# YuliangXiu/ICON

Hardware: NVIDIA H100
Metric: M query-points/sec at 256^3 grid (higher is better)
Workload: dtype f32

## Files before the change

icon_b200/_C.py:

```python
import ctypes
import os

_HERE = os.path.dirname(os.path.abspath(__file__))
LIB_PATH = os.environ.get("ICON_B200_LIB") or os.path.join(_HERE, "libicon_b200.so")

if not os.path.exists(LIB_PATH):
    raise ImportError(
        f"{LIB_PATH} is missing: the CUDA extension must be built (python -m icon_b200.build); "
        "icon_b200 has no CPU or PyTorch fallback.")

lib = ctypes.CDLL(LIB_PATH)

_vp, _i, _i64, _f, _sz = ctypes.c_void_p, ctypes.c_int, ctypes.c_int64, ctypes.c_float, ctypes.c_size_t

_SIGS = {
    "icon_version": (_i, []),
    "icon_last_error": (ctypes.c_char_p, []),
    "icon_launch_count": (_i64, []),
    "icon_profile_enable": (_i, [_i]),
    "icon_profile_last_query": (_i, [_vp]),
    "icon_smpl_workspace_bytes": (_sz, [_i, _i]),
    "icon_smpl_prepare": (_i, [_vp, _vp, _vp, _vp, _i, _i, _vp, _sz, _vp]),
    "icon_query_workspace_bytes": (_sz, [_i64, _i, _i]),
    "icon_set_mlp_impl": (_i, [_i]),
    "icon_get_mlp_impl": (_i, []),
    "icon_query": (_i, [_i, _vp, _i64, _i64, _i64, _vp, _vp, _i, _i, _i, _vp, _i, _vp, _i, _i, _vp, _vp, _i, _f,
                        _vp, _vp, _sz, _vp]),
    "icon_query_feats": (_i, [_i, _vp, _i64, _i64, _i64, _vp, _vp, _i, _i, _i, _vp, _i, _vp, _i, _i, _vp, _vp, _i, _f,
                              _i, _vp, _vp, _sz, _vp]),
    "icon_set_sdf_policy": (_i, [_i, _i64, _i64]),
    "icon_set_sdf_bricks": (_i, [_i, _i64]),
    "icon_sdf_brick_info": (_i, [_vp, _i, _i, _vp]),
    "icon_sdf_brick_lists": (_i, [_vp, _i, _i, _vp, _vp, _vp, _vp, _vp, _vp, _vp]),
    "icon_sdf_only": (_i, [_vp, _i64, _i64, _i64, _vp, _vp, _i, _i, _vp, _vp, _vp, _sz, _vp]),
    "icon_sdf_bruteforce": (_i, [_vp, _i64, _i64, _i64, _vp, _vp, _i, _i, _vp, _vp, _vp]),
    "icon_face_tree_read": (_i, [_vp, _i, _i, _vp, _vp, _vp, _vp]),
    "icon_mesh_workspace_bytes": (_sz, [_i, _i]),
    "icon_mesh_prepare": (_i, [_vp, _vp, _i, _i, _vp, _sz, _vp]),
    "icon_mesh_distance": (_i, [_vp, _i64, _vp, _i, _i, _vp, _vp, _vp]),
    "icon_mesh_sample_workspace_bytes": (_sz, [_i]),
    "icon_mesh_sample": (_i, [_vp, _vp, _i, _i, _vp, _i, ctypes.c_uint64, _vp, _vp, _vp, _vp, _sz, _vp]),
    "icon_prt_workspace_bytes": (_sz, [_i, _i, _i]),
    "icon_prt": (_i, [_vp, _i, _i, _vp, _vp, _i, ctypes.c_double, _vp, _vp, _i, _i, ctypes.c_double, _vp, _vp, _vp, _sz,
                      _vp]),
    "icon_mlp_only": (_i, [_vp, _i, _i64, _vp, _vp, _vp, _vp]),
    "icon_display": (_i, [_vp, _i, _vp, _vp]),
    "icon_grid_upsample": (_i, [_vp, _vp, _i, _f, _vp, _vp, _vp, _vp]),
    "icon_grid_dilate": (_i, [_vp, _i, _i, _vp, _vp, _vp]),
    "icon_compact_workspace_bytes": (_sz, [_i]),
    "icon_grid_compact": (_i, [_vp, _vp, _i, _i, _vp, _vp, _vp, _vp, _i64, _vp, _vp, _sz, _vp]),
    "icon_grid_scatter": (_i, [_vp, _vp, _vp, _i64, _vp]),
    "icon_grid_init_points": (_i, [_i, _i, _vp, _vp, _vp, _vp]),
    "icon_grid_count_above": (_i, [_vp, _i64, _f, _vp, _vp]),
    "icon_conv_nhwc_workspace_bytes": (_sz, [_i, _i, _i, _i, _i]),
    "icon_conv_nhwc": (_i, [_vp, _vp, _vp, _vp, _vp, _i, _vp, _vp, _vp, _i, _i, _i, _i, _i, _i, _i, _i, _i, _i, _i, _i, _i,
                           _i, _vp, _i, _i, _i, _vp, _vp, _sz, _vp]),
    "icon_norm_finalize": (_i, [_vp, _vp, _vp, _vp, _i, _i, _i, ctypes.c_double, _f, _vp]),
    "icon_act_nhwc": (_i, [_vp, _i, _i, _vp, _vp, _vp, _vp, _i, _f, _vp, _vp, _vp, _vp, _i, _i, _i, _i, _i, _i, _i, _i, _vp]),
    "icon_splitk_instnorm_act": (_i, [_vp, _i, _vp, _vp, _vp, _vp, _vp, _i, _i, _i, _i, _i, _i, _i, _f, _vp]),
    "icon_col2im7": (_i, [_vp, _vp, _vp, _i, _i, _i, _i, _i, _i, _vp]),
    "icon_ew_nhwc": (_i, [_i, _vp, _vp, _vp, _vp, _vp, _i, _i, _i, _i, _vp]),
    "icon_nchw_to_nhwc": (_i, [_vp, _vp, _vp, _i, _i, _i64, _vp]),
    "icon_nhwc_to_nchw": (_i, [_vp, _vp, _i, _i, _i, _i, _i64, _vp]),
    "icon_stem_pack": (_i, [_vp, _vp, _vp, _i, _i, _i, _i, _i, _i, _i, _i, _i, _vp]),
    "icon_clean_mesh_workspace_bytes": (_sz, [_i64, _i64]),
    "icon_clean_mesh_count": (_i, [_vp, _i64, _i64, _vp, _sz, _vp, _vp]),
    "icon_clean_mesh_emit": (_i, [_vp, _i, _vp, _i64, _i64, _vp, _vp, _vp, _vp]),
    "icon_conv3d": (_i, [_vp, _vp, _vp, _vp, _vp, _vp, _i, _i, _i, _i, _i, _i, _i, _i, _i, _i, _vp]),
    "icon_normalize_mask": (_i, [_vp, _vp, _vp, _i, _i, _i64, _vp]),
    "icon_voxelize_workspace_bytes": (_sz, [_i]),
    "icon_voxelize": (_i, [_vp, _i, _i, _vp, _vp, _i, _i, _f, _vp, _vp, _sz, _vp]),
    "icon_visibility_workspace_bytes": (_sz, [_i]),
    "icon_visibility": (_i, [_vp, _i, _vp, _i, _i, _vp, _vp, _sz, _vp]),
    "icon_vertex_normals_workspace_bytes": (_sz, [_i, _i]),
    "icon_vertex_normals": (_i, [_vp, _i, _vp, _i, _vp, _vp, _sz, _vp]),
    "icon_normal_render_workspace_bytes": (_sz, [_i, _i, _i, _i]),
    "icon_normal_render": (_i, [_vp, _vp, _i, _vp, _i, _vp, _i, _i, _vp, _vp, _vp, _sz, _vp]),
    "icon_dataset_render_workspace_bytes": (_sz, [_i, _i, _i, _i]),
    "icon_dataset_render": (_i, [_vp, _vp, _i, _i, _i, _vp, _vp, _sz, _vp]),
    "icon_dataset_texture_bytes": (_sz, [_i, _i]),
    "icon_dataset_texture": (_i, [_vp, _i, _i, _vp, _sz, _vp]),
    "icon_area_vertex_normals_workspace_bytes": (_sz, [_i, _i]),
    "icon_area_vertex_normals": (_i, [_vp, _i, _vp, _i, _vp, _vp, _sz, _vp]),
    "icon_area_vertex_normals_backward_workspace_bytes": (_sz, [_i, _i]),
    "icon_area_vertex_normals_backward": (_i, [_vp, _i, _vp, _i, _vp, _vp, _vp, _sz, _vp]),
    "icon_mesh_topology_workspace_bytes": (_sz, [_i, _i]),
    "icon_mesh_topology_count": (_i, [_vp, _i, _i, ctypes.POINTER(_i64), _vp, _sz, _vp]),
    "icon_mesh_topology_build": (_i, [_vp, _vp, _sz, _vp]),
    "icon_vertex_edges_workspace_bytes": (_sz, [_i, _i]),
    "icon_vertex_edges": (_i, [_vp, _i, _i, _vp, _vp, _vp, _sz, _vp]),
    "icon_mesh_priors_workspace_bytes": (_sz, [_i, _i, _i, _i]),
    "icon_mesh_priors_forward": (_i, [_vp, _vp, _vp, _vp, _vp, _vp, _sz, _vp]),
    "icon_mesh_priors_backward": (_i, [_vp, _vp, _vp, _vp, _vp, _vp, _vp, _sz, _vp]),
    "icon_local_affine_forward": (_i, [_vp, _vp, _vp, _i, _vp, _i, _vp, _vp, _vp, _vp]),
    "icon_local_affine_backward": (_i, [_vp, _vp, _vp, _i, _vp, _i, _vp, _vp, _vp, _vp, _vp, _vp, _vp, _vp, _vp]),
    "icon_mesh_views_workspace_bytes": (_sz, [_i, _i, _i, _i]),
    "icon_mesh_views": (_i, [_vp, _vp, _i, _vp, _i, _vp, _i, _i, _vp, _vp, _vp, _vp, _sz, _vp]),
    "icon_mesh_render_state_bytes": (_sz, [_i, _i, _i]),
    "icon_mesh_render_workspace_bytes": (_sz, [_i, _i, _i, _i, _i, _i]),
    "icon_mesh_render_forward": (_i, [_i, _vp, _vp, _i, _vp, _i, _vp, _i, _i, _vp, _vp, _sz, _vp, _sz, _vp]),
    "icon_mesh_render_backward": (_i, [_i, _vp, _vp, _i, _vp, _i, _vp, _i, _i, _vp, _vp, _sz, _vp, _vp, _vp, _sz,
                                       _vp]),
    "icon_lbs_prepare_workspace_bytes": (_sz, [_i, _i, _i]),
    "icon_lbs_prepare": (_i, [_vp, _vp, _i, _vp, _sz, _vp]),
    "icon_lbs_state_bytes": (_sz, [_i, _i, _i, _i]),
    "icon_lbs_workspace_bytes": (_sz, [_i, _i, _i, _i, _i]),
    "icon_lbs_forward": (_i, [_vp, _i, _vp, _vp, _i, _vp, _vp, _vp, _sz, _vp, _sz, _vp]),
    "icon_lbs_backward": (_i, [_vp, _i, _vp, _sz, _vp, _vp, _vp, _vp, _vp, _sz, _vp]),
    "icon_smplx_heads_prepare": (_i, [_vp, _vp, _i, _vp, _vp, _i, _vp, _vp, _i, _vp, _vp, _i, _vp, _vp, _i, _vp, _i,
                                      _vp]),
    "icon_smplx_heads_state_bytes": (_sz, [_i, _i, _i]),
    "icon_smplx_heads_forward": (_i, [_vp, _i, _vp, _vp, _vp, _vp, _vp, _vp, _vp, _sz, _vp]),
    "icon_smplx_heads_backward": (_i, [_vp, _i, _vp, _vp, _vp, _vp, _vp, _vp]),
    "icon_tetra_prepare": (_i, [_vp, _vp, _i, _i, _i]),
    "icon_tetra_state_bytes": (_sz, []),
    "icon_tetra_forward": (_i, [_vp, _vp, _vp, _vp, _vp, _vp, _vp, _vp, _sz, _vp]),
    "icon_remesh_workspace_bytes": (_sz, [_i, _i, _i]),
    "icon_remesh_compact": (_i, [_vp, _i, _vp, _i, _vp, _vp, _vp, _vp, _sz, _vp]),
    "icon_remesh_classify": (_i, [_vp, _vp, _vp, _sz, _vp]),
    "icon_remesh_smooth_step": (_i, [_vp, _vp, _vp, _vp, _sz, _vp]),
    "icon_remesh_midpoints": (_i, [_vp, _vp, _vp, _vp]),
    "icon_remesh_select": (_i, [_i, _vp, _vp, ctypes.c_double, _i, _vp, ctypes.c_double, _vp, _vp, _sz, _vp]),
    "icon_remesh_apply": (_i, [_i, _vp, _vp, _i, _vp, _vp, _vp, _sz, _vp]),
    "icon_remesh_relax": (_i, [_vp, _vp, _vp, _vp, _vp, _vp, _vp, _sz, _vp]),
    "icon_remesh_reproject": (_i, [_vp, _i, _vp, _vp, _vp, _vp, _vp, _vp]),
    "icon_mc_workspace_bytes": (_sz, [_i, _i]),
    "icon_mc_count": (_i, [_vp, _i, ctypes.c_double, _i, _vp, _sz, _vp, _vp]),
    "icon_mc_emit": (_i, [_vp, _i, ctypes.c_double, _i, _vp, _vp, _vp, _i64, _i64, _vp]),
    "icon_garment_labels_workspace_bytes": (_sz, [_i]),
    "icon_garment_labels": (_i, [_vp, _i, _vp, _i, _vp, _vp, _vp, _sz, _vp]),
    "icon_garment_face_mask_workspace_bytes": (_sz, [_i, _i]),
    "icon_garment_face_mask": (_i, [_vp, _i, _vp, _i, _vp, ctypes.c_uint32, _vp, _i, _vp, _i, _vp, _vp, _vp, _sz,
                                    _vp]),
}

EXPORTS = tuple(_SIGS.keys())

for _name, (_res, _args) in _SIGS.items():
    _fn = getattr(lib, _name)
    _fn.restype = _res
    _fn.argtypes = _args


class MeshTopology(ctypes.Structure):
    _fields_ = [("V", _i), ("F", _i), ("E", _i), ("faces", _vp), ("edges", _vp), ("face_to_edge", _vp),
                ("vert_off", _vp), ("vert_edges", _vp), ("edge_off", _vp), ("edge_entries", _vp),
                ("corner_off", _vp), ("vert_corners", _vp)]


class LbsModel(ctypes.Structure):
    _fields_ = [("V", _i), ("J", _i), ("NB", _i), ("parents", _i * 64), ("v_template", _vp), ("shapedirs", _vp),
                ("posedirs", _vp), ("J_regressor", _vp), ("lbs_weights", _vp), ("J_template", _vp), ("J_dirs", _vp)]


class SmplxHeads(ctypes.Structure):
    _fields_ = [("V", _i), ("J", _i), ("R", _i), ("Ls", _i), ("Ld", _i), ("E", _i), ("nchain", _i),
                ("chain", _i * 8), ("regressor", _vp), ("vid", _vp), ("bc", _vp), ("joint_reg", _vp),
                ("reg_joint", _vp), ("inc_off", _vp), ("inc", _vp)]


class TetraModel(ctypes.Structure):
    _fields_ = [("V", _i), ("N", _i), ("T", _i), ("nnz", _i), ("parents", _i * 24), ("v_template", _vp),
                ("shapedirs", _vp), ("posedirs", _vp), ("weights", _vp), ("jr_off", _vp), ("jr_col", _vp),
                ("jr_val", _vp)]


class DatasetMesh(ctypes.Structure):
    _fields_ = [("mode", _i), ("F", _i), ("V", _i), ("Vn", _i), ("Vt", _i), ("Va", _i), ("pos", _vp), ("nrm", _vp),
                ("uv", _vp), ("attr", _vp), ("f_pos", _vp), ("f_nrm", _vp), ("f_uv", _vp), ("f_attr", _vp),
                ("tex", _vp), ("tex_w", _i), ("tex_h", _i)]


class IconError(RuntimeError):
    pass


def check(rc, what):
    if rc != 0:
        msg = lib.icon_last_error().decode("utf-8", "replace")
        raise IconError(f"{what} failed (code {rc}): {msg}")


def launch_count():
    return int(lib.icon_launch_count())
```

icon_b200/csrc/mlp.cu:

```cuda
#include "common.cuh"
#include "query_common.cuh"

namespace icon {

constexpr int MP = 64;
constexpr int MT = 256;
constexpr int KC = 16;

constexpr int OFF_W0 = 0;
constexpr int OFF_B0 = OFF_W0 + 16 * 512;
constexpr int OFF_W1 = OFF_B0 + 512;
constexpr int OFF_B1 = OFF_W1 + 512 * 256;
constexpr int OFF_W2 = OFF_B1 + 256;
constexpr int OFF_B2 = OFF_W2 + 272 * 128;
constexpr int OFF_W3 = OFF_B2 + 128;
constexpr int OFF_B3 = OFF_W3 + 144;
static_assert(OFF_B3 + 1 == ICON_MLP_PACKED_FLOATS, "packed layout");

template <int MODE>
__global__ void __launch_bounds__(MT, 2) k_query_mlp(QueryParams q) {
    extern __shared__ __align__(16) float sm[];
    float *x0s = sm;
    float *stage = sm + 16 * MP;
    float *h1s = stage + 10240;
    float *w1c = stage;
    float *h0c = stage + 2 * KC * 256;
    float *w2c = stage;
    float *red = stage + 2 * KC * 128;

    const int tid = threadIdx.x;
    const int64_t p0 = (int64_t)blockIdx.x * MP;
    const float *__restrict__ W = q.mlp;
    const int c0 = q.c0;

    {
        const float4 *src = (const float4 *)(W + OFF_W1);
        for (int i = tid; i < KC * 256 / 4; i += MT) cp_async16(w1c + 4 * i, src + i);
        cp_async_commit();
    }

    {
        const int pl = tid & (MP - 1), grp = tid >> 6;
        const int64_t pi = p0 + pl;
        const bool live = pi < q.N;
        if (MODE == 3) {
            for (int r = grp; r < 16; r += 4) x0s[r * MP + pl] = (live && r < c0) ? q.raw[(size_t)r * q.N + pi] : 0.f;
        } else {
            float4 xyz = live ? q.xyz4[pi] : make_float4(0.f, 0.f, 0.f, 0.f);
            if (MODE == 0) {
                const bool has_vis = q.feats & ICON_FEAT_VIS;
                const int d = has_vis ? q.C / 2 : q.C;
                float4 r0 = make_float4(0.f, 0.f, 0.f, 0.f), r1 = r0;
                if (live) {
                    const float4 *r = (const float4 *)(q.rec + 8 * pi);
                    r0 = r[0]; r1 = r[1];
                }
                const float vis = r1.w;
                if (grp == 0) {
                    float sdf = r0.x, cx = r0.y, cy = r0.z, cz = r0.w;
                    const bool outlier = live && fabsf(sdf) >= q.clip;
                    if (outlier) sdf = sdf > 0.f ? 1.f : -1.f;
                    int col = d;
                    x0s[col++ * MP + pl] = sdf;
                    if (q.feats & ICON_FEAT_CMAP) {
                        if (outlier) {
                            long long K = *q.d_K;
                            long long k3 = 3ll * (long long)q.krank[pi];
                            cx = (float)q.signs[(k3) % K];
                            cy = (float)q.signs[(k3 + 1) % K];
                            cz = (float)q.signs[(k3 + 2) % K];
                        }
                        x0s[col++ * MP + pl] = cx;
                        x0s[col++ * MP + pl] = cy;
                        x0s[col++ * MP + pl] = cz;
                    }
                    if (q.feats & ICON_FEAT_NORM) {
                        x0s[col++ * MP + pl] = r1.x;
                        x0s[col++ * MP + pl] = r1.y;
                        x0s[col++ * MP + pl] = r1.z;
                    }
                    for (int r = col; r < 16; ++r) x0s[r * MP + pl] = 0.f;
                } else {
                    const int base = !has_vis || vis != 0.f ? 0 : d;
                    for (int ch = grp - 1; ch < d; ch += 3) {
                        float v = live ? bilinear(q.feat + (size_t)(base + ch) * q.H * q.W, q.H, q.W, xyz.x, xyz.y) : 0.f;
                        x0s[ch * MP + pl] = v;
                    }
                }
            } else if (MODE == 1) {
                for (int ch = grp; ch < q.C; ch += 4) {
                    float v = live ? bilinear(q.feat + (size_t)ch * q.H * q.W, q.H, q.W, xyz.x, xyz.y) : 0.f;
                    x0s[ch * MP + pl] = v;
                }
                if (grp == 0) {
                    x0s[q.C * MP + pl] = live ? xyz.z : 0.f;
                    for (int r = q.C + 1; r < 16; ++r) x0s[r * MP + pl] = 0.f;
                }
            } else {
                if (grp < 3) {
                    for (int ch = grp; ch < q.C; ch += 3) {
                        float v = live ? bilinear(q.feat + (size_t)ch * q.H * q.W, q.H, q.W, xyz.x, xyz.y) : 0.f;
                        x0s[ch * MP + pl] = v;
                    }
                } else {
                    const size_t vs = (size_t)q.VD * q.VD * q.VD;
                    for (int ch = 0; ch < 7; ++ch) {
                        float v = live ? trilinear(q.vol + ch * vs, q.VD, xyz.x, xyz.y, xyz.z) : 0.f;
                        x0s[(q.C + ch) * MP + pl] = v;
                    }
                    for (int r = q.C + 7; r < 16; ++r) x0s[r * MP + pl] = 0.f;
                }
            }
        }
    }
    __syncthreads();

    const int ty = tid >> 3, tx = tid & 7;
    float acc[8][8];
#pragma unroll
    for (int i = 0; i < 8; ++i)
#pragma unroll
        for (int j = 0; j < 8; ++j) acc[i][j] = 0.f;

    const int hc = tid >> 4, hp = tid & 15;

    constexpr int NST1 = 512 / KC;
    for (int st = 0; st < NST1; ++st) {
        const int buf = st & 1;
        {
            const int ch = st * KC + hc;
            float a0 = __ldg(W + OFF_B0 + ch), a1 = a0, a2 = a0, a3 = a0;
#pragma unroll
            for (int j = 0; j < 16; ++j) {
                float w = __ldg(W + OFF_W0 + j * 512 + ch);
                float4 xv = *(const float4 *)(x0s + j * MP + hp * 4);
                a0 = fmaf(w, xv.x, a0); a1 = fmaf(w, xv.y, a1); a2 = fmaf(w, xv.z, a2); a3 = fmaf(w, xv.w, a3);
            }
            *(float4 *)(h0c + buf * KC * MP + hc * MP + hp * 4) = make_float4(lrelu(a0), lrelu(a1), lrelu(a2), lrelu(a3));
        }
        if (st + 1 < NST1) {
            const float4 *src = (const float4 *)(W + OFF_W1 + (size_t)(st + 1) * KC * 256);
            float *dst = w1c + (buf ^ 1) * KC * 256;
            for (int i = tid; i < KC * 256 / 4; i += MT) cp_async16(dst + 4 * i, src + i);
            cp_async_commit();
            cp_async_wait<1>();
        } else {
            cp_async_wait<0>();
        }
        __syncthreads();
        const float *wb = w1c + buf * KC * 256 + ty * 8;
        const float *hb = h0c + buf * KC * MP + tx * 4;
#pragma unroll
        for (int k = 0; k < KC; ++k) {
            float4 a0 = *(const float4 *)(wb + k * 256), a1 = *(const float4 *)(wb + k * 256 + 4);
            float4 b0 = *(const float4 *)(hb + k * MP), b1 = *(const float4 *)(hb + k * MP + 32);
            float a[8] = {a0.x, a0.y, a0.z, a0.w, a1.x, a1.y, a1.z, a1.w};
            float b[8] = {b0.x, b0.y, b0.z, b0.w, b1.x, b1.y, b1.z, b1.w};
#pragma unroll
            for (int i = 0; i < 8; ++i)
#pragma unroll
                for (int j = 0; j < 8; ++j) acc[i][j] = fmaf(a[i], b[j], acc[i][j]);
        }
        __syncthreads();
    }
#pragma unroll
    for (int i = 0; i < 8; ++i) {
        const int ch = ty * 8 + i;
        const float bia = __ldg(W + OFF_B1 + ch);
        *(float4 *)(h1s + ch * MP + tx * 4) = make_float4(lrelu(acc[i][0] + bia), lrelu(acc[i][1] + bia),
                                                         lrelu(acc[i][2] + bia), lrelu(acc[i][3] + bia));
        *(float4 *)(h1s + ch * MP + 32 + tx * 4) = make_float4(lrelu(acc[i][4] + bia), lrelu(acc[i][5] + bia),
                                                              lrelu(acc[i][6] + bia), lrelu(acc[i][7] + bia));
    }
    {
        const float4 *src = (const float4 *)(W + OFF_W2);
        for (int i = tid; i < KC * 128 / 4; i += MT) cp_async16(w2c + 4 * i, src + i);
        cp_async_commit();
    }
    __syncthreads();

    float acc2[4][8];
#pragma unroll
    for (int i = 0; i < 4; ++i)
#pragma unroll
        for (int j = 0; j < 8; ++j) acc2[i][j] = 0.f;
    constexpr int NST2 = 272 / KC;
    for (int st = 0; st < NST2; ++st) {
        const int buf = st & 1;
        if (st + 1 < NST2) {
            const float4 *src = (const float4 *)(W + OFF_W2 + (size_t)(st + 1) * KC * 128);
            float *dst = w2c + (buf ^ 1) * KC * 128;
            for (int i = tid; i < KC * 128 / 4; i += MT) cp_async16(dst + 4 * i, src + i);
            cp_async_commit();
            cp_async_wait<1>();
        } else {
            cp_async_wait<0>();
        }
        __syncthreads();
        const float *wb = w2c + buf * KC * 128 + ty * 4;
        const float *hb = (st < 16 ? h1s + (size_t)st * KC * MP : x0s) + tx * 4;
#pragma unroll
        for (int k = 0; k < KC; ++k) {
            float4 a0 = *(const float4 *)(wb + k * 128);
            float4 b0 = *(const float4 *)(hb + k * MP), b1 = *(const float4 *)(hb + k * MP + 32);
            float a[4] = {a0.x, a0.y, a0.z, a0.w};
            float b[8] = {b0.x, b0.y, b0.z, b0.w, b1.x, b1.y, b1.z, b1.w};
#pragma unroll
            for (int i = 0; i < 4; ++i)
#pragma unroll
                for (int j = 0; j < 8; ++j) acc2[i][j] = fmaf(a[i], b[j], acc2[i][j]);
        }
        __syncthreads();
    }

    float part[8];
#pragma unroll
    for (int j = 0; j < 8; ++j) part[j] = 0.f;
#pragma unroll
    for (int i = 0; i < 4; ++i) {
        const int ch = ty * 4 + i;
        const float bia = __ldg(W + OFF_B2 + ch), w3 = __ldg(W + OFF_W3 + ch);
#pragma unroll
        for (int j = 0; j < 8; ++j) part[j] = fmaf(w3, lrelu(acc2[i][j] + bia), part[j]);
    }
#pragma unroll
    for (int j = 0; j < 8; ++j) {
        part[j] += __shfl_xor_sync(0xffffffffu, part[j], 8);
        part[j] += __shfl_xor_sync(0xffffffffu, part[j], 16);
    }
    const int lane = tid & 31, wid = tid >> 5;
    if (lane < 8) {
#pragma unroll
        for (int j = 0; j < 4; ++j) {
            red[wid * MP + lane * 4 + j] = part[j];
            red[wid * MP + 32 + lane * 4 + j] = part[4 + j];
        }
    }
    __syncthreads();
    if (tid < MP) {
        const int64_t pi = p0 + tid;
        if (pi < q.N) {
            float s = 0.f;
#pragma unroll
            for (int w = 0; w < 8; ++w) s += red[w * MP + tid];
            for (int j = 0; j < 16; ++j) s = fmaf(__ldg(W + OFF_W3 + 128 + j), x0s[j * MP + tid], s);
            s += __ldg(W + OFF_B3);
            float in_cube = (MODE == 3) ? 1.f : q.xyz4[pi].w;
            q.out[pi] = in_cube * s;
        }
    }
}

__global__ void k_outlier_flag(const float *__restrict__ rec, int64_t N, float clip, int32_t *__restrict__ flag) {
    int64_t i = (int64_t)blockIdx.x * blockDim.x + threadIdx.x;
    if (i < N) flag[i] = fabsf(rec[8 * i]) >= clip ? 1 : 0;
}
__global__ void k_outlier_signs(const float *__restrict__ rec, int64_t N, float clip,
                                const int32_t *__restrict__ krank, int8_t *__restrict__ signs) {
    int64_t i = (int64_t)blockIdx.x * blockDim.x + threadIdx.x;
    if (i < N) {
        float s = rec[8 * i];
        if (fabsf(s) >= clip) signs[krank[i]] = s > 0.f ? 1 : -1;
    }
}

constexpr size_t MLP_SMEM = (16 * MP + 10240 + 256 * MP) * sizeof(float);

template <int MODE>
static int launch_mlp(const QueryParams &q, cudaStream_t stream) {
    static bool attr_set[ICON_MAX_DEVICES] = {};
    if (device_needs_setup(attr_set))
        ICON_CUDA(cudaFuncSetAttribute(k_query_mlp<MODE>, cudaFuncAttributeMaxDynamicSharedMemorySize, (int)MLP_SMEM));
    unsigned nblk = (unsigned)((q.N + MP - 1) / MP);
    k_query_mlp<MODE><<<nblk, MT, MLP_SMEM, stream>>>(q);
    ICON_LAUNCHED();
    return ICON_OK;
}

int launch_mlp_tc(int mode, const QueryParams &q, const void *blob, cudaStream_t stream);
static int g_mlp_impl = 1;

template <int MODE>
static int launch_any(const QueryParams &q, const void *tc, cudaStream_t stream) {
    if (g_mlp_impl == 1) {
        if (!tc) {
            set_error("icon_query / icon_mlp_only: the tensor-core MLP needs the packed tensor-core weight blob (mlp_tc == NULL); "
                      "pass it or select the FP32 kernel with icon_set_mlp_impl(0)");
            return ICON_EINVAL;
        }
        if (q.c0 > 15) {
            set_error("icon_query / icon_mlp_only: the tensor-core MLP takes c0 <= 15 input channels (got %d)", q.c0);
            return ICON_EINVAL;
        }
        return launch_mlp_tc(MODE, q, tc, stream);
    }
    return launch_mlp<MODE>(q, stream);
}

size_t sdf_ws_bytes(int64_t N);
int run_sdf(const float *points, int64_t sc, int64_t sn, int64_t N, const float *h_calib, const MeshView &m,
            float *rec, int32_t *face, void *ws, float4 **xyz4_out, cudaStream_t stream);
int run_points_only(const float *points, int64_t sc, int64_t sn, int64_t N, const float *h_calib,
                    float4 *xyz4, cudaStream_t stream);

struct QueryWs {
    void *sdf_ws;
    float *rec;
    int32_t *krank;
    int8_t *signs;
    int64_t *d_K;
    void *scan_ws;
    float4 *xyz4;
};

static QueryWs carve_query(Carver &c, int64_t N, int prior) {
    QueryWs w{};
    if (prior == ICON_PRIOR_ICON) {
        w.sdf_ws = c.take<char>(sdf_ws_bytes(N));
        w.rec = c.take<float>((size_t)N * 8);
        w.krank = c.take<int32_t>((size_t)N);
        w.signs = c.take<int8_t>((size_t)N);
        w.d_K = c.take<int64_t>(1);
        w.scan_ws = c.take<char>(scan_ws_bytes(N));
    } else {
        w.xyz4 = c.take<float4>((size_t)N);
    }
    return w;
}

}

using namespace icon;

extern "C" size_t icon_query_workspace_bytes(int64_t N, int F, int prior) {
    (void)F;
    Carver c(nullptr);
    carve_query(c, N, prior);
    return c.total();
}

extern "C" int icon_query(int prior, const float *points, int64_t stride_c, int64_t stride_n, int64_t N,
                          const float *h_calib, const float *feat, int C, int H, int W,
                          const float *vol_feat, int VD, const void *mesh_ws, int V, int F,
                          const float *mlp_packed, const void *mlp_tc, int c0, float sdf_clip, float *out,
                          void *ws, size_t ws_bytes, icon_stream_t stream) {
    return icon_query_feats(prior, points, stride_c, stride_n, N, h_calib, feat, C, H, W, vol_feat, VD, mesh_ws, V, F,
                            mlp_packed, mlp_tc, c0, sdf_clip, ICON_FEAT_ALL, out, ws, ws_bytes, stream);
}

extern "C" int icon_query_feats(int prior, const float *points, int64_t stride_c, int64_t stride_n, int64_t N,
                                const float *h_calib, const float *feat, int C, int H, int W,
                                const float *vol_feat, int VD, const void *mesh_ws, int V, int F,
                                const float *mlp_packed, const void *mlp_tc, int c0, float sdf_clip, int smpl_feats,
                                float *out, void *ws, size_t ws_bytes, icon_stream_t stream_) {
    cudaStream_t stream = (cudaStream_t)stream_;
    ICON_CHECK_ARG(N >= 0 && N < (int64_t)INT32_MAX, "icon_query: N=%lld out of range", (long long)N);
    if (N == 0) return ICON_OK;
    ICON_CHECK_ARG(points && h_calib && feat && mlp_packed && out && ws, "icon_query: null pointer");
    ICON_CHECK_ARG(((uintptr_t)mlp_tc & 15) == 0, "icon_query: mlp_tc must be 16-byte aligned");
    ICON_CHECK_ARG(c0 >= 1 && c0 <= 16, "icon_query: c0=%d unsupported (1..16)", c0);
    ICON_CHECK_ARG(H >= 2 && W >= 2, "icon_query: feature map %dx%d too small", H, W);
    {
        Carver c(nullptr);
        carve_query(c, N, prior);
        if (ws_bytes < c.total()) {
            set_error("icon_query: workspace %zu < %zu", ws_bytes, c.total());
            return ICON_ENOSPC;
        }
    }
    Carver c(ws);
    QueryWs w = carve_query(c, N, prior);
    QueryParams q{};
    q.feat = feat; q.C = C; q.H = H; q.W = W; q.vol = vol_feat; q.VD = VD;
    q.mlp = mlp_packed; q.c0 = c0; q.clip = sdf_clip; q.out = out; q.N = N;
    if (prior == ICON_PRIOR_ICON) {
        ICON_CHECK_ARG(mesh_ws && V > 0 && F > 0, "icon_query: icon prior needs a prepared body mesh");
        ICON_CHECK_ARG((smpl_feats & ~ICON_FEAT_ALL) == 0, "icon_query: smpl_feats mask %d has bits outside ICON_FEAT_ALL",
                       smpl_feats);
        const int cm = smpl_feats & ICON_FEAT_CMAP ? 1 : 0, nm = smpl_feats & ICON_FEAT_NORM ? 1 : 0;
        const bool vs = smpl_feats & ICON_FEAT_VIS;
        const int tail = 1 + 3 * cm + 3 * nm;
        ICON_CHECK_ARG((!vs || C % 2 == 0) && c0 == (vs ? C / 2 : C) + tail,
                       "icon_query: icon prior with smpl_feats mask %d expects c0 = %s + %d (C=%d c0=%d)", smpl_feats,
                       vs ? "C/2" : "C", tail, C, c0);
        q.feats = smpl_feats;
        MeshView m = mesh_view(mesh_ws, V, F);
        float4 *xyz4 = nullptr;
        int rc = run_sdf(points, stride_c, stride_n, N, h_calib, m, w.rec, nullptr, w.sdf_ws, &xyz4, stream);
        if (rc) return rc;
        if (cm) {
            unsigned nb = (unsigned)((N + 255) / 256);
            k_outlier_flag<<<nb, 256, 0, stream>>>(w.rec, N, sdf_clip, w.krank);
            ICON_LAUNCHED();
            rc = scan_exclusive_i32(w.krank, w.krank, N, w.d_K, w.scan_ws, stream);
            if (rc) return rc;
            k_outlier_signs<<<nb, 256, 0, stream>>>(w.rec, N, sdf_clip, w.krank, w.signs);
            ICON_LAUNCHED();
            q.krank = w.krank; q.signs = w.signs; q.d_K = w.d_K;
        }
        q.xyz4 = xyz4; q.rec = w.rec;
        profile_mark(3, stream);
        rc = launch_any<0>(q, mlp_tc, stream);
        profile_mark(4, stream);
        return rc;
    }
    profile_mark(0, stream);
    int rc = run_points_only(points, stride_c, stride_n, N, h_calib, w.xyz4, stream);
    if (rc) return rc;
    profile_mark(1, stream); profile_mark(2, stream); profile_mark(3, stream);
    q.xyz4 = w.xyz4;
    if (prior == ICON_PRIOR_PIFU) {
        ICON_CHECK_ARG(C + 1 == c0, "icon_query: pifu prior expects c0 = C + 1 (C=%d c0=%d)", C, c0);
        rc = launch_any<1>(q, mlp_tc, stream);
        profile_mark(4, stream);
        return rc;
    }
    if (prior == ICON_PRIOR_PAMIR) {
        ICON_CHECK_ARG(vol_feat && VD >= 2 && C + 7 == c0, "icon_query: pamir prior expects vol_feat and c0 = C + 7");
        rc = launch_any<2>(q, mlp_tc, stream);
        profile_mark(4, stream);
        return rc;
    }
    set_error("icon_query: unknown prior %d", prior);
    return ICON_EINVAL;
}

extern "C" int icon_set_mlp_impl(int impl) {
    ICON_CHECK_ARG(impl == 0 || impl == 1, "icon_set_mlp_impl: 0 (fp32) or 1 (tensor cores)");
    g_mlp_impl = impl;
    return ICON_OK;
}
extern "C" int icon_get_mlp_impl(void) { return g_mlp_impl; }

extern "C" int icon_mlp_only(const float *feature, int c0, int64_t N, const float *mlp_packed, const void *mlp_tc,
                             float *out, icon_stream_t stream_) {
    cudaStream_t stream = (cudaStream_t)stream_;
    if (N == 0) return ICON_OK;
    ICON_CHECK_ARG(feature && mlp_packed && out && c0 >= 1 && c0 <= 16, "icon_mlp_only: bad argument");
    QueryParams q{};
    q.raw = feature; q.mlp = mlp_packed; q.c0 = c0; q.out = out; q.N = N;
    return launch_any<3>(q, mlp_tc, stream);
}
```

icon_b200/csrc/mlp_tc.cu:

```cuda
#include <cuda_fp16.h>

#include "common.cuh"
#include "query_common.cuh"
#include "wgmma.cuh"

namespace icon {

constexpr int TC_THREADS = 384;
constexpr int TC_M = 128;
constexpr int NSTAGE = 4;
constexpr int STAGE_BYTES = 32768;
constexpr int STAGES_PER_TILE = 20;
static_assert(STAGES_PER_TILE % NSTAGE == 0 && NSTAGE % 2 == 0, "layer-1 hi / lo pairs must stay on stages (2i, 2i + 1)");
constexpr int GATHER_THREADS = 96;

constexpr int TCB_W0 = 0;
constexpr int TCB_W1 = 32768;
constexpr int TCB_W2 = TCB_W1 + 8 * 65536;
constexpr int TCB_W2T = TCB_W2 + 4 * 32768;
constexpr int TCB_F32 = TCB_W2T + 8192;
constexpr int TCB_F32_FLOATS = 512 + 256 + 128 + 144 + 4;
constexpr int TCB_BYTES = TCB_F32 + TCB_F32_FLOATS * 4;
static_assert(TCB_BYTES == ICON_MLP_TC_BYTES, "blob layout");

constexpr int SM_STAGE = 0;
constexpr int SM_W0 = NSTAGE * STAGE_BYTES;
constexpr int SM_X0 = SM_W0 + 32768;
constexpr int X0_H = 0;
constexpr int X0_L = 4096;
constexpr int X0_F = 8192;
constexpr int X0_SLOT = 16384;
constexpr int SM_F32 = SM_X0 + 2 * X0_SLOT;
constexpr int SM_W2T = (SM_F32 + TCB_F32_FLOATS * 4 + 127) / 128 * 128;
constexpr int SM_BAR = SM_W2T + 8192;
constexpr int NBAR = 2 * NSTAGE + 5;
constexpr int SM_TOTAL = SM_BAR + NBAR * 8;
constexpr int TC_SMEM_BYTES = SM_TOTAL + 1024;
static_assert(TC_SMEM_BYTES <= 227 * 1024, "shared memory");

enum { B_FULL0 = 0, B_EMPTY0 = NSTAGE, B_W0RDY = 2 * NSTAGE, B_XFULL0 = 2 * NSTAGE + 1, B_XEMPTY0 = 2 * NSTAGE + 3 };

constexpr int REG_CONSUMER = 224, REG_PRODUCER = 56;
static_assert(2 * 128 * REG_CONSUMER + 128 * REG_PRODUCER <= 168 * TC_THREADS, "register split");

__device__ __forceinline__ void act_frag64(const float *d, const float *bias, uint32_t (&ah)[4][4], uint32_t (&al)[4][4]) {
#pragma unroll
    for (int kk = 0; kk < 4; ++kk) {
#pragma unroll
        for (int q = 0; q < 4; ++q) {
            const int nb = 2 * kk + (q >> 1), e = 4 * nb + 2 * (q & 1);
            float v0 = d[e], v1 = d[e + 1];
            if (bias) { v0 += bias[8 * nb]; v1 += bias[8 * nb + 1]; }
            v0 = fmaxf(v0, 0.01f * v0); v1 = fmaxf(v1, 0.01f * v1);
            wg::split2(v0, v1, ah[kk][q], al[kk][q]);
        }
    }
}

template <int MODE>
__device__ __forceinline__ void gather_point(const QueryParams &q, int64_t pi, float *xf) {
#pragma unroll
    for (int j = 0; j < 15; ++j) xf[j * TC_M] = 0.f;
    float in_cube = 1.f;
    if (pi < q.N) {
        if (MODE == 3) {
            const int c0 = q.c0;
#pragma unroll
            for (int j = 0; j < 15; ++j)
                if (j < c0) xf[j * TC_M] = q.raw[(size_t)j * q.N + pi];
        } else {
            const float4 xyz = q.xyz4[pi];
            in_cube = xyz.w;
            if (MODE == 0) {
                const bool has_vis = q.feats & ICON_FEAT_VIS;
                const int d = has_vis ? q.C / 2 : q.C;
                const float4 *rp = (const float4 *)(q.rec + 8 * pi);
                const float4 r0 = rp[0], r1 = rp[1];
                const int fb = has_vis && r1.w == 0.f ? d : 0;
                float sdf = r0.x;
                const bool outlier = fabsf(sdf) >= q.clip;
                if (outlier) sdf = sdf > 0.f ? 1.f : -1.f;
                float *col = xf + d * TC_M;
                col[0] = sdf;
                col += TC_M;
                if (q.feats & ICON_FEAT_CMAP) {
                    float cx = r0.y, cy = r0.z, cz = r0.w;
                    if (outlier) {
                        const long long K = *q.d_K, k3 = 3ll * (long long)q.krank[pi];
                        cx = (float)q.signs[k3 % K];
                        cy = (float)q.signs[(k3 + 1) % K];
                        cz = (float)q.signs[(k3 + 2) % K];
                    }
                    col[0] = cx; col[TC_M] = cy; col[2 * TC_M] = cz;
                    col += 3 * TC_M;
                }
                if (q.feats & ICON_FEAT_NORM) { col[0] = r1.x; col[TC_M] = r1.y; col[2 * TC_M] = r1.z; }
                if (d == 6) {
#pragma unroll
                    for (int ch = 0; ch < 6; ++ch)
                        xf[ch * TC_M] = bilinear(q.feat + (size_t)(fb + ch) * q.H * q.W, q.H, q.W, xyz.x, xyz.y);
                } else {
#pragma unroll
                    for (int ch = 0; ch < 14; ++ch)
                        if (ch < d) xf[ch * TC_M] = bilinear(q.feat + (size_t)(fb + ch) * q.H * q.W, q.H, q.W, xyz.x, xyz.y);
                }
            } else if (MODE == 1) {
                if (q.C == 12) {
#pragma unroll
                    for (int ch = 0; ch < 12; ++ch)
                        xf[ch * TC_M] = bilinear(q.feat + (size_t)ch * q.H * q.W, q.H, q.W, xyz.x, xyz.y);
                } else {
#pragma unroll
                    for (int ch = 0; ch < 14; ++ch)
                        if (ch < q.C) xf[ch * TC_M] = bilinear(q.feat + (size_t)ch * q.H * q.W, q.H, q.W, xyz.x, xyz.y);
                }
                if (q.C < 15) xf[q.C * TC_M] = xyz.z;
            } else {
                const size_t vs = (size_t)q.VD * q.VD * q.VD;
                if (q.C == 6) {
#pragma unroll
                    for (int ch = 0; ch < 6; ++ch)
                        xf[ch * TC_M] = bilinear(q.feat + (size_t)ch * q.H * q.W, q.H, q.W, xyz.x, xyz.y);
                } else {
#pragma unroll
                    for (int ch = 0; ch < 8; ++ch)
                        if (ch < q.C) xf[ch * TC_M] = bilinear(q.feat + (size_t)ch * q.H * q.W, q.H, q.W, xyz.x, xyz.y);
                }
#pragma unroll
                for (int ch = 0; ch < 7; ++ch)
                    if (q.C + ch < 15) xf[(q.C + ch) * TC_M] = trilinear(q.vol + ch * vs, q.VD, xyz.x, xyz.y, xyz.z);
            }
        }
    }
    xf[15 * TC_M] = in_cube;
}

template <int MODE>
__global__ void __launch_bounds__(TC_THREADS, 1) k_query_mlp_tc(QueryParams q, const uint8_t *__restrict__ blob) {
    using namespace wg;
    extern __shared__ uint8_t smem_raw[];
    const uint32_t raw = s32(smem_raw);
    const uint32_t base = (raw + 1023u) & ~1023u;
    uint8_t *sm = smem_raw + (base - raw);
    const float *sf32 = reinterpret_cast<const float *>(sm + SM_F32);
    const float *sb1 = sf32 + 512, *sw3 = sf32 + 896, *sb3 = sf32 + 1040;
    const uint32_t bar0 = base + SM_BAR;
    auto BAR = [&](int i) { return bar0 + 8u * (uint32_t)i; };

    const int tid = threadIdx.x, warp = tid >> 5, lane = tid & 31;
    const int64_t ntiles = (q.N + TC_M - 1) / TC_M;

    if (tid == 0) {
        for (int s = 0; s < NSTAGE; ++s) { mbar_init(BAR(B_FULL0 + s), 1); mbar_init(BAR(B_EMPTY0 + s), 8); }
        mbar_init(BAR(B_W0RDY), 1);
        for (int b = 0; b < 2; ++b) { mbar_init(BAR(B_XFULL0 + b), GATHER_THREADS); mbar_init(BAR(B_XEMPTY0 + b), 8); }
        asm volatile("fence.mbarrier_init.release.cluster;" ::: "memory");
    }
    __syncthreads();

    if (warp >= 8) {
        asm volatile("setmaxnreg.dec.sync.aligned.u32 %0;" ::"n"(REG_PRODUCER));
        if (warp == 8) {
            if (lane == 0) {
                mbar_expect_tx(BAR(B_W0RDY), 32768 + TCB_F32_FLOATS * 4 + 8192);
                bulk_g2s(base + SM_W0, blob + TCB_W0, 32768, BAR(B_W0RDY));
                bulk_g2s(base + SM_F32, blob + TCB_F32, TCB_F32_FLOATS * 4, BAR(B_W0RDY));
                bulk_g2s(base + SM_W2T, blob + TCB_W2T, 8192, BAR(B_W0RDY));
                uint32_t cnt = 0;
                for (int64_t tile = blockIdx.x; tile < ntiles; tile += gridDim.x) {
                    for (int i = 0; i < STAGES_PER_TILE; ++i, ++cnt) {
                        const uint32_t s = cnt % NSTAGE, ph = (cnt / NSTAGE) & 1;
                        mbar_wait(BAR(B_EMPTY0 + s), ph ^ 1);
                        const uint32_t dst = base + SM_STAGE + s * STAGE_BYTES, full = BAR(B_FULL0 + s);
                        mbar_expect_tx(full, STAGE_BYTES);
                        const uint8_t *src = i < 16 ? blob + TCB_W1 + (size_t)i * 32768 : blob + TCB_W2 + (size_t)(i - 16) * 32768;
                        bulk_g2s(dst, src, STAGE_BYTES, full);
                    }
                }
            }
        } else {
            const int gt = tid - 9 * 32;
            for (uint32_t it = 0; blockIdx.x + (int64_t)it * gridDim.x < ntiles; ++it) {
                const int b = it & 1;
                mbar_wait(BAR(B_XEMPTY0 + b), ((it >> 1) & 1) ^ 1);
                uint8_t *xs = sm + SM_X0 + b * X0_SLOT;
                for (int r = gt; r < TC_M; r += GATHER_THREADS) {
                    float *xf = reinterpret_cast<float *>(xs + X0_F) + r;
                    gather_point<MODE>(q, (blockIdx.x + (int64_t)it * gridDim.x) * TC_M + r, xf);
                    uint32_t hi[8], lo[8];
#pragma unroll
                    for (int i = 0; i < 7; ++i) split2(xf[2 * i * TC_M], xf[(2 * i + 1) * TC_M], hi[i], lo[i]);
                    split2(xf[14 * TC_M], 1.f, hi[7], lo[7]);
                    const int off = (r >> 3) * 128 + (r & 7) * 16;
                    *reinterpret_cast<uint4 *>(xs + X0_H + off) = make_uint4(hi[0], hi[1], hi[2], hi[3]);
                    *reinterpret_cast<uint4 *>(xs + X0_H + off + 2048) = make_uint4(hi[4], hi[5], hi[6], hi[7]);
                    *reinterpret_cast<uint4 *>(xs + X0_L + off) = make_uint4(lo[0], lo[1], lo[2], lo[3]);
                    *reinterpret_cast<uint4 *>(xs + X0_L + off + 2048) = make_uint4(lo[4], lo[5], lo[6], lo[7]);
                }
                fence_proxy_async();
                mbar_arrive(BAR(B_XFULL0 + b));
            }
        }
        return;
    }

    asm volatile("setmaxnreg.inc.sync.aligned.u32 %0;" ::"n"(REG_CONSUMER));
    const int g = warp >> 2;
    const int rf = 64 * g + 16 * (warp & 3) + (lane >> 2);
    const int cq = 2 * (lane & 3);
    uint32_t cnt = 0;
    auto stage_wait = [&](uint32_t c) {
        const uint32_t s = c % NSTAGE;
        mbar_wait(BAR(B_FULL0 + s), (c / NSTAGE) & 1);
        return s;
    };
    auto warp_arrive = [&](int bar) {
        __syncwarp();
        if (lane == 0) mbar_arrive(BAR(bar));
    };
    const uint64_t dw2th = desc_nosw(base + SM_W2T, 2048, 128), dw2tl = desc_nosw(base + SM_W2T + 4096, 2048, 128);
    mbar_wait(BAR(B_W0RDY), 0);

    uint32_t it = 0;
    for (int64_t tile = blockIdx.x; tile < ntiles; tile += gridDim.x, ++it) {
        const int b = it & 1;
        const uint32_t xs = base + SM_X0 + b * X0_SLOT;
        const uint64_t dx0h = desc_nosw(xs + X0_H + g * 1024, 2048, 128), dx0l = desc_nosw(xs + X0_L + g * 1024, 2048, 128);
        mbar_wait(BAR(B_XFULL0 + b), (it >> 1) & 1);

        auto layer0 = [&](int j, float (&a0)[32]) {
            const uint64_t w0h = desc_nosw(base + SM_W0 + j * 1024, 8192, 128), w0l = w0h + (16384 >> 4);
            fence();
            mma_ss<64>(a0, dx0h, w0h, 0);
            mma_ss<64>(a0, dx0h, w0l, 1);
            mma_ss<64>(a0, dx0l, w0h, 1);
            commit();
        };
        float acc1[128];
        auto layer1 = [&](int j, uint32_t (&ch)[4][4], uint32_t (&cl)[4][4], uint32_t (&nh)[4][4], uint32_t (&nl)[4][4]) {
            wait<0>();
            if (j) { warp_arrive(B_EMPTY0 + (cnt - 2) % NSTAGE); warp_arrive(B_EMPTY0 + (cnt - 1) % NSTAGE); }
            float a0[32];
            if (j < 7) layer0(j + 1, a0);
            const uint32_t s = stage_wait(cnt);
            stage_wait(cnt + 1);
            const uint64_t bh = desc_sw128(base + SM_STAGE + s * STAGE_BYTES), bl = bh + (STAGE_BYTES >> 4);
            fence();
#pragma unroll
            for (int kk = 0; kk < 4; ++kk) {
                mma_rs<256>(acc1, ch[kk], bh + 2 * kk, (j | kk) != 0);
                mma_rs<256>(acc1, ch[kk], bl + 2 * kk, 1);
                mma_rs<256>(acc1, cl[kk], bh + 2 * kk, 1);
            }
            commit();
            cnt += 2;
            if (j < 7) {
                wait<1>();
                fence_regs(a0);
                act_frag64(a0, nullptr, nh, nl);
            }
        };
        uint32_t xh[4][4], xl[4][4], yh[4][4], yl[4][4];
        {
            float a0[32];
            layer0(0, a0);
            wait<0>();
            fence_regs(a0);
            act_frag64(a0, nullptr, xh, xl);
        }
#pragma unroll
        for (int j = 0; j < 8; j += 2) {
            layer1(j, xh, xl, yh, yl);
            layer1(j + 1, yh, yl, xh, xl);
        }
        wait<0>();
        fence_regs(acc1);
        warp_arrive(B_EMPTY0 + (cnt - 2) % NSTAGE);
        warp_arrive(B_EMPTY0 + (cnt - 1) % NSTAGE);

        float acc2[64];
        auto layer2 = [&](int c, uint32_t (&ch)[4][4], uint32_t (&cl)[4][4]) {
            const uint32_t s = stage_wait(cnt);
            const uint64_t bh = desc_sw128(base + SM_STAGE + s * STAGE_BYTES), bl = bh + (16384 >> 4);
            fence();
#pragma unroll
            for (int kk = 0; kk < 4; ++kk) {
                mma_rs<128>(acc2, ch[kk], bh + 2 * kk, (c | kk) != 0);
                mma_rs<128>(acc2, ch[kk], bl + 2 * kk, 1);
                mma_rs<128>(acc2, cl[kk], bh + 2 * kk, 1);
            }
            commit();
            ++cnt;
            if (c) {
                wait<1>();
                warp_arrive(B_EMPTY0 + (cnt - 2) % NSTAGE);
            }
        };
        act_frag64(acc1, sb1 + cq, xh, xl);
        layer2(0, xh, xl);
        act_frag64(acc1 + 32, sb1 + 64 + cq, yh, yl);
        layer2(1, yh, yl);
        act_frag64(acc1 + 64, sb1 + 128 + cq, xh, xl);
        layer2(2, xh, xl);
        act_frag64(acc1 + 96, sb1 + 192 + cq, yh, yl);
        layer2(3, yh, yl);
        fence();
        mma_ss<128>(acc2, dx0h, dw2th, 1);
        mma_ss<128>(acc2, dx0h, dw2tl, 1);
        mma_ss<128>(acc2, dx0l, dw2th, 1);
        commit();
        wait<0>();
        fence_regs(acc2);
        warp_arrive(B_EMPTY0 + (cnt - 1) % NSTAGE);

        const float *x0f = reinterpret_cast<const float *>(sm + (xs - base) + X0_F);
        float s0 = 0.f, s1 = 0.f;
#pragma unroll
        for (int i = 0; i < 16; ++i) {
            const float w0 = sw3[8 * i + cq], w1 = sw3[8 * i + cq + 1];
            float v0 = acc2[4 * i], v1 = acc2[4 * i + 1], v2 = acc2[4 * i + 2], v3 = acc2[4 * i + 3];
            v0 = fmaxf(v0, 0.01f * v0); v1 = fmaxf(v1, 0.01f * v1);
            v2 = fmaxf(v2, 0.01f * v2); v3 = fmaxf(v3, 0.01f * v3);
            s0 = fmaf(w0, v0, s0); s0 = fmaf(w1, v1, s0);
            s1 = fmaf(w0, v2, s1); s1 = fmaf(w1, v3, s1);
        }
        s0 += __shfl_xor_sync(0xffffffffu, s0, 1); s0 += __shfl_xor_sync(0xffffffffu, s0, 2);
        s1 += __shfl_xor_sync(0xffffffffu, s1, 1); s1 += __shfl_xor_sync(0xffffffffu, s1, 2);
        if ((lane & 3) < 2) {
            const int r = rf + 8 * (lane & 1);
            float s = (lane & 1) ? s1 : s0;
            const int64_t pi = tile * TC_M + r;
            if (pi < q.N) {
#pragma unroll
                for (int j = 0; j < 15; ++j) s = fmaf(sw3[128 + j], x0f[j * TC_M + r], s);
                s += sb3[0];
                q.out[pi] = x0f[15 * TC_M + r] != 0.f ? s : copysignf(0.f, s);
            }
        }
        warp_arrive(B_XEMPTY0 + b);
    }
}

template <int MODE>
int launch_mlp_tc_t(const QueryParams &q, const void *blob, cudaStream_t stream) {
    static bool attr_set[ICON_MAX_DEVICES] = {};
    if (device_needs_setup(attr_set)) {
        ICON_CUDA(cudaFuncSetAttribute(k_query_mlp_tc<MODE>, cudaFuncAttributeMaxDynamicSharedMemorySize, TC_SMEM_BYTES));
    }

    const int sms = device_sm_count();
    const int64_t ntiles = (q.N + TC_M - 1) / TC_M;
    const unsigned grid = (unsigned)(ntiles < sms ? ntiles : sms);
    k_query_mlp_tc<MODE><<<grid, TC_THREADS, TC_SMEM_BYTES, stream>>>(q, (const uint8_t *)blob);
    ICON_LAUNCHED();
    return ICON_OK;
}

int launch_mlp_tc(int mode, const QueryParams &q, const void *blob, cudaStream_t stream) {
    switch (mode) {
        case 0: return launch_mlp_tc_t<0>(q, blob, stream);
        case 1: return launch_mlp_tc_t<1>(q, blob, stream);
        case 2: return launch_mlp_tc_t<2>(q, blob, stream);
        default: return launch_mlp_tc_t<3>(q, blob, stream);
    }
}

}
```

icon_b200/csrc/query_common.cuh:

```cuda
#pragma once
#include "common.cuh"

namespace icon {

struct QueryParams {
    const float4 *xyz4;
    const float *rec;
    const int32_t *krank;
    const int8_t *signs;
    const int64_t *d_K;
    int feats;
    const float *feat;
    int C, H, W;
    const float *vol;
    int VD;
    const float *raw;
    const float *mlp;
    int c0;
    float clip;
    float *out;
    int64_t N;
};

__device__ __forceinline__ float lrelu(float x) { return x > 0.f ? x : 0.01f * x; }

__device__ __forceinline__ void cp_async16(void *smem, const void *gmem) {
    unsigned s = (unsigned)__cvta_generic_to_shared(smem);
    asm volatile("cp.async.cg.shared.global [%0], [%1], 16;\n" ::"r"(s), "l"(gmem));
}
__device__ __forceinline__ void cp_async_commit() { asm volatile("cp.async.commit_group;\n" ::); }
template <int N>
__device__ __forceinline__ void cp_async_wait() { asm volatile("cp.async.wait_group %0;\n" ::"n"(N)); }

__device__ __forceinline__ float bilinear(const float *__restrict__ plane, int H, int W, float x, float y) {
    float ix = ((x + 1.f) / 2.f) * (float)(W - 1);
    float iy = ((y + 1.f) / 2.f) * (float)(H - 1);
    float fx = floorf(ix), fy = floorf(iy);
    int x0 = (int)fx, y0 = (int)fy, x1 = x0 + 1, y1 = y0 + 1;
    float wx1 = ix - fx, wy1 = iy - fy, wx0 = (fx + 1.f) - ix, wy0 = (fy + 1.f) - iy;
    float o = 0.f;
    bool vx0 = x0 >= 0 && x0 < W, vx1 = x1 >= 0 && x1 < W, vy0 = y0 >= 0 && y0 < H, vy1 = y1 >= 0 && y1 < H;
    if (vx0 && vy0) o += __ldg(plane + (size_t)y0 * W + x0) * (wx0 * wy0);
    if (vx1 && vy0) o += __ldg(plane + (size_t)y0 * W + x1) * (wx1 * wy0);
    if (vx0 && vy1) o += __ldg(plane + (size_t)y1 * W + x0) * (wx0 * wy1);
    if (vx1 && vy1) o += __ldg(plane + (size_t)y1 * W + x1) * (wx1 * wy1);
    return o;
}

__device__ __forceinline__ float trilinear(const float *__restrict__ v, int D, float x, float y, float z) {
    float ix = ((x + 1.f) / 2.f) * (float)(D - 1);
    float iy = ((y + 1.f) / 2.f) * (float)(D - 1);
    float iz = ((z + 1.f) / 2.f) * (float)(D - 1);
    float fx = floorf(ix), fy = floorf(iy), fz = floorf(iz);
    int x0 = (int)fx, y0 = (int)fy, z0 = (int)fz;
    float tx = ix - fx, ty = iy - fy, tz = iz - fz;
    float o = 0.f;
#pragma unroll
    for (int dz = 0; dz < 2; ++dz)
#pragma unroll
        for (int dy = 0; dy < 2; ++dy)
#pragma unroll
            for (int dx = 0; dx < 2; ++dx) {
                int xx = x0 + dx, yy = y0 + dy, zz = z0 + dz;
                if (xx >= 0 && xx < D && yy >= 0 && yy < D && zz >= 0 && zz < D) {
                    float w = (dx ? tx : 1.f - tx) * (dy ? ty : 1.f - ty) * (dz ? tz : 1.f - tz);
                    o += __ldg(v + ((size_t)zz * D + yy) * D + xx) * w;
                }
            }
    return o;
}

}
```

icon_b200/csrc/sdf.cu:

```cuda
#include <float.h>

#include <algorithm>
#include <mutex>
#include <type_traits>
#include <unordered_set>
#include <vector>

#include "common.cuh"
#include "face_tree.cuh"
#include "geom.cuh"

namespace icon {

struct Calib {
    float r[9];
    float t[3];
};

__device__ __forceinline__ V3 load_point(const float *__restrict__ pts, int64_t sc, int64_t sn,
                                         int64_t i, const Calib &cb) {
    float px = pts[i * sn], py = pts[sc + i * sn], pz = pts[2 * sc + i * sn];
    V3 o;
    o.x = fmaf(cb.r[2], pz, fmaf(cb.r[1], py, cb.r[0] * px)) + cb.t[0];
    o.y = fmaf(cb.r[5], pz, fmaf(cb.r[4], py, cb.r[3] * px)) + cb.t[1];
    o.z = fmaf(cb.r[8], pz, fmaf(cb.r[7], py, cb.r[6] * px)) + cb.t[2];
    return o;
}

__device__ __forceinline__ void emit_record(V3 p, int bi, float best, int hits, const MeshView &m,
                                            float *__restrict__ rec, int32_t *__restrict__ face,
                                            int64_t idx) {
    Tri t = load_tri(m.tri + 3 * (size_t)bi);
    V3 n = cross3(t.ab, t.ac);
    float s = n.x * n.x + n.y * n.y + n.z * n.z;
    if (s == 0.f) s = 1e-6f;
    float inv = 1.0f / s;
    V3 w = sub3(p, t.a);
    V3 uw = cross3(t.ab, w), wv = cross3(w, t.ac);
    float b2 = (uw.x * n.x + uw.y * n.y + uw.z * n.z) * inv;
    float b1 = (wv.x * n.x + wv.y * n.y + wv.z * n.z) * inv;
    float b0 = 1.0f - b1 - b2;
    const float4 *at = m.attr + 6 * (size_t)bi;
    float4 a0 = __ldg(at), a1 = __ldg(at + 1), a2 = __ldg(at + 2), a3 = __ldg(at + 3),
           a4 = __ldg(at + 4), a5 = __ldg(at + 5);
    float nx = (a0.x * b0 + a0.w * b1 + a1.z * b2) * -1.f;
    float ny = (a0.y * b0 + a1.x * b1 + a1.w * b2) * 1.f;
    float nz = (a0.z * b0 + a1.y * b1 + a2.x * b2) * -1.f;
    float cx = a2.y * b0 + a3.x * b1 + a3.w * b2;
    float cy = a2.z * b0 + a3.y * b1 + a4.x * b2;
    float cz = a2.w * b0 + a3.z * b1 + a4.y * b2;
    float vv = a4.z * b0 + a4.w * b1 + a5.x * b2;
    float vis = vv >= 0.1f ? 1.f : 0.f;
    float dist = sqrtf(best) / sqrtf(3.0f);
    float sign = 2.0f * ((float)(hits & 1) - 0.5f);
    float sdf = dist * sign;
    float4 *r = (float4 *)(rec + 8 * idx);
    r[0] = make_float4(sdf, cx, cy, cz);
    r[1] = make_float4(nx, ny, nz, vis);
    if (face) face[idx] = bi;
}

constexpr int SW_T = 128;
constexpr int NBIN_AX = 128;
constexpr int NBIN = NBIN_AX * NBIN_AX * NBIN_AX;
__host__ __device__ constexpr int fr_cap(int ppw) { return ppw >= 16 ? 1024 : (ppw >= 4 ? 768 : 384); }

__device__ __forceinline__ unsigned spread7(unsigned v) {
    v = (v | (v << 16)) & 0x030000FFu;
    v = (v | (v << 8)) & 0x0300F00Fu;
    v = (v | (v << 4)) & 0x030C30C3u;
    v = (v | (v << 2)) & 0x09249249u;
    return v;
}

__device__ __forceinline__ int bin_of(V3 p) {
    const bool inside = p.x >= -1.f && p.x <= 1.f && p.y >= -1.f && p.y <= 1.f && p.z >= -1.f && p.z <= 1.f;
    if (!inside) return NBIN;
    const unsigned bx = min(NBIN_AX - 1, (int)((p.x + 1.f) * (NBIN_AX * 0.5f)));
    const unsigned by = min(NBIN_AX - 1, (int)((p.y + 1.f) * (NBIN_AX * 0.5f)));
    const unsigned bz = min(NBIN_AX - 1, (int)((p.z + 1.f) * (NBIN_AX * 0.5f)));
    return (int)(spread7(bx) | (spread7(by) << 1) | (spread7(bz) << 2));
}

__global__ void k_points_bin(const float *__restrict__ pts, int64_t sc, int64_t sn, int64_t N, Calib cb,
                             float4 *__restrict__ xyz4, int32_t *__restrict__ bid, int32_t *__restrict__ count) {
    const int64_t i = (int64_t)blockIdx.x * blockDim.x + threadIdx.x;
    const bool live = i < N;
    int b = -1;
    if (live) {
        const V3 p = load_point(pts, sc, sn, i, cb);
        const float in_cube = (p.x > -1.f && p.x < 1.f && p.y > -1.f && p.y < 1.f && p.z > -1.f && p.z < 1.f) ? 1.f : 0.f;
        xyz4[i] = make_float4(p.x, p.y, p.z, in_cube);
        b = bin_of(p);
        bid[i] = b;
    }
    const unsigned act = __ballot_sync(0xffffffffu, live);
    if (live) {
        const unsigned peers = __match_any_sync(act, b);
        if ((int)(threadIdx.x & 31) == __ffs(peers) - 1) atomicAdd(&count[b], __popc(peers));
    }
}

__global__ void k_points_scatter(const int32_t *__restrict__ bid, int64_t N, const int32_t *__restrict__ offset,
                                 int32_t *__restrict__ cursor, int32_t *__restrict__ perm) {
    const int64_t i = (int64_t)blockIdx.x * blockDim.x + threadIdx.x;
    const bool live = i < N;
    const int b = live ? bid[i] : -1;
    const unsigned act = __ballot_sync(0xffffffffu, live);
    if (live) {
        const unsigned peers = __match_any_sync(act, b);
        const int lane = threadIdx.x & 31, leader = __ffs(peers) - 1;
        int base = 0;
        if (lane == leader) base = atomicAdd(&cursor[b], __popc(peers));
        base = __shfl_sync(peers, base, leader);
        perm[offset[b] + base + __popc(peers & ((1u << lane) - 1u))] = (int32_t)i;
    }
}

#ifdef ICON_SDF_STATS
__device__ unsigned long long g_stats[8];
__device__ unsigned *g_wstat;
enum { WS_DEFER, WS_ENTRIES, WS_STEPS, WS_STAGED, WS_SPH, WS_EXACT, WS_WIN, WS_RAY, WS_CYC_START, WS_CYC_C,
       WS_CYC_RAY, WS_CYC_EMIT, WS_UB0, WS_UBEND, WS_LIST, WS_IDEAL_ENTRIES, WS_IDEAL_FACES, WS_DEAD, WS_N = 20 };
#define STAT(i, v) do { if (lane == 0) atomicAdd(&g_stats[i], (unsigned long long)(v)); } while (0)
#define WSTAT(i, v) do { if (lane == 0 && g_wstat) g_wstat[(size_t)wid * WS_N + (i)] = (unsigned)(v); } while (0)
#define WCLK(t) __syncwarp(); const long long t = clock64()
#else
#define STAT(i, v) do { } while (0)
#define WSTAT(i, v) do { } while (0)
#endif

template <int PPW, bool BRICK>
using SdfSmem = typename std::conditional<BRICK, ChunkSmem, WalkSmem<unsigned short, fr_cap(PPW)>>::type;
template <int PPW, bool BRICK>
constexpr size_t sdf_smem_bytes() { return sizeof(SdfSmem<PPW, BRICK>) * (SW_T / 32); }

constexpr float BRICK_W = 2.0f / BRICK_AX;
constexpr float BRICK_HALF_DIAG = 0.0541266f;

__device__ __forceinline__ void brick_box(int b, float4 &lo, float4 &hi) {
    const int bx = b % BRICK_AX, by = (b / BRICK_AX) % BRICK_AX, bz = b / (BRICK_AX * BRICK_AX);
    lo = make_float4(-1.f + bx * BRICK_W, -1.f + by * BRICK_W, -1.f + bz * BRICK_W, 0.f);
    hi = make_float4(-1.f + (bx + 1) * BRICK_W, -1.f + (by + 1) * BRICK_W, -1.f + (bz + 1) * BRICK_W, 0.f);
}

__device__ __forceinline__ float leaf_key(const MeshView &m, int l, float4 lo, float4 hi) {
    const float4 a = __ldg(m.nodes + 2 * (size_t)l), z = __ldg(m.nodes + 2 * (size_t)l + 1);
    const float gx = fmaxf(fmaxf(a.x - hi.x, lo.x - z.x), 0.f);
    const float gy = fmaxf(fmaxf(a.y - hi.y, lo.y - z.y), 0.f);
    const float gz = fmaxf(fmaxf(a.z - hi.z, lo.z - z.z), 0.f);
    return fmaf(gz, gz, fmaf(gy, gy, gx * gx));
}

template <int PPW, bool BRICK>
__device__ __forceinline__ void sdf_warp(int64_t wid, SdfSmem<PPW, BRICK> &S, const float4 *__restrict__ xyz4,
                                         const int32_t *__restrict__ perm, int64_t N, const MeshView &m,
                                         float *__restrict__ rec, int32_t *__restrict__ face,
                                         int32_t *__restrict__ defer, int32_t *__restrict__ ndefer) {
    constexpr int REP = 32 / PPW;
    const int lane = threadIdx.x & 31;
    const int sub = lane % PPW, rep_id = lane / PPW;
    const int64_t pos0 = wid * PPW;
    const int64_t pos = pos0 + sub;
    if (pos0 >= N) return;
    const bool live = pos < N;
    const int64_t idx = perm[live ? pos : pos0];
    const float4 q = xyz4[idx];
    const V3 p = mk3(q.x, q.y, q.z);
    const V3 c = mk3(0.5f * (warp_min(p.x) + warp_max(p.x)), 0.5f * (warp_min(p.y) + warp_max(p.y)),
                     0.5f * (warp_min(p.z) + warp_max(p.z)));
    const float rw = warp_max(sqrtf(dot3(sub3(p, c), sub3(p, c)))) * 1.00001f + 1e-6f;
    const float4 wlo = make_float4(warp_min(p.x) - 1e-6f, warp_min(p.y) - 1e-6f, warp_min(p.z) - 1e-6f, 0.f);
    const float4 whi = make_float4(warp_max(p.x) + 1e-6f, warp_max(p.y) + 1e-6f, warp_max(p.z) + 1e-6f, 0.f);
    const MeshHeader h = *m.hdr;

    NearestFace<PPW> nf(p, 1e-6f, 1e-7f);
#ifdef ICON_SDF_STATS
    WCLK(t_start);
    long long t_c = 0, t_ray = 0;
    int st_entries = 0, st_steps = 0, st_brick = -1;
    float st_ub0 = 0.f;
#endif
    if constexpr (BRICK) {
        bool ok = h.brick_built && !h.brick_overflow && c.x >= -1.f && c.x < 1.f && c.y >= -1.f && c.y < 1.f &&
                  c.z >= -1.f && c.z < 1.f;
        int b = 0;
        float4 blo, bhi;
        if (ok) {
            const int bx = min(BRICK_AX - 1, (int)((c.x + 1.f) * (BRICK_AX * 0.5f)));
            const int by = min(BRICK_AX - 1, (int)((c.y + 1.f) * (BRICK_AX * 0.5f)));
            const int bz = min(BRICK_AX - 1, (int)((c.z + 1.f) * (BRICK_AX * 0.5f)));
            b = (bz * BRICK_AX + by) * BRICK_AX + bx;
            brick_box(b, blo, bhi);
            ok = wlo.x >= blo.x && wlo.y >= blo.y && wlo.z >= blo.z && whi.x <= bhi.x && whi.y <= bhi.y && whi.z <= bhi.z;
        }
        if (!ok) {
            if (lane == 0) defer[atomicAdd(ndefer, 1)] = (int32_t)wid;
            WSTAT(WS_DEFER, 1);
            return;
        }
        const int f = __ldg(m.bface + b);
        nf.try_face(m.tri + 3 * (size_t)f, f);
        nf.start_scan(fminf(warp_max(sqrtf(nf.best)), __ldg(m.bub + b)), wlo, whi);
        STAT(0, 1);
#ifdef ICON_SDF_STATS
        WCLK(t_c0);
        t_c = t_c0;
        st_brick = b;
        st_ub0 = nf.ub;
#endif
        const int o1 = __ldg(m.foff + b + 1);
        for (int base = __ldg(m.foff + b); base < o1; base += 32) {
            const int slot = base + lane;
            const bool in = slot < o1;
            const int k = in ? (int)__ldg(m.flist + slot) : -1;
            const float key = in ? __ldg(m.fkey + slot) : 0.f;
            if (__shfl_sync(0xffffffffu, key, 0) > nf.ub * nf.ub) break;
            STAT(2, min(32, o1 - base));
#ifdef ICON_SDF_STATS
            st_entries += min(32, o1 - base);
            ++st_steps;
#endif
            nf.chunk(m, S, k, wlo, whi);
        }
        nf.merge();
    } else {
        const int n = tree_nearest(m, S, nf, c, rw, wlo, whi);
        STAT(0, 1); STAT(1, n > fr_cap(PPW) ? 1 : 0); STAT(2, n);
    }
    STAT(3, nf.staged);
#ifdef ICON_SDF_STATS
    WCLK(t_c1);
    int st_ray = 0;
#endif
    int hits = 0;
    if (!h.ray_overflow) {
        const float fy = (p.y - h.y0) * h.inv_cy, fz = (p.z - h.z0) * h.inv_cz;
        if (fy >= 0.f && fy < (float)RAY_GRID && fz >= 0.f && fz < (float)RAY_GRID) {
            const int cc = (int)fz * RAY_GRID + (int)fy;
            const int k0 = __ldg(m.roff + cc), k1 = __ldg(m.roff + cc + 1);
            for (int k = k0 + rep_id; k < k1; k += REP) {
                const int f = __ldg(m.rlist + k);
                if (__ldg(&m.rbox[2 * (size_t)f + 1].x) < p.x - 1e-3f) continue;
                const Tri tr = load_tri(m.tri + 3 * (size_t)f);
                hits += ray_hit_px(p, tr.a, tr.ab, tr.ac);
#ifdef ICON_SDF_STATS
                ++st_ray;
#endif
            }
        }
    } else {
        for (int f = rep_id; f < m.F; f += REP) {
            const Tri tr = load_tri(m.tri + 3 * (size_t)f);
            hits += ray_hit_px(p, tr.a, tr.ab, tr.ac);
        }
    }
    if (REP > 1) {
#pragma unroll
        for (int o = PPW; o < 32; o <<= 1) hits += __shfl_xor_sync(0xffffffffu, hits, o);
    }
#ifdef ICON_SDF_STATS
    WCLK(t_ray0);
    t_ray = t_ray0;
#endif
    if (live && rep_id == 0) emit_record(p, nf.bi, nf.best, hits, m, rec, face, idx);
#ifdef ICON_SDF_STATS
    WCLK(t_end);
    if (BRICK && st_brick >= 0) {
        const float ube = nf.ub;
        int il = 0, ifc = 0;
        const int o0 = __ldg(m.foff + st_brick), o1 = __ldg(m.foff + st_brick + 1);
        for (int s = o0 + lane; s < o1; s += 32) {
            il += __ldg(m.fkey + s) <= ube * ube;
            const float4 s4 = __ldg(m.sph_s + __ldg(m.flist + s));
            const float l2 = ube + s4.w;
            ifc += box_dist2(mk3(s4.x, s4.y, s4.z), wlo, whi) <= l2 * l2;
        }
        const int s_sph = __reduce_add_sync(0xffffffffu, nf.n_sph), s_exact = __reduce_add_sync(0xffffffffu, nf.n_exact);
        const int s_win = __reduce_add_sync(0xffffffffu, nf.n_win), s_ray = __reduce_add_sync(0xffffffffu, st_ray);
        const int s_il = __reduce_add_sync(0xffffffffu, il), s_if = __reduce_add_sync(0xffffffffu, ifc);
        WSTAT(WS_ENTRIES, st_entries);
        WSTAT(WS_STEPS, st_steps);
        WSTAT(WS_STAGED, nf.staged);
        WSTAT(WS_SPH, s_sph);
        WSTAT(WS_EXACT, s_exact);
        WSTAT(WS_WIN, s_win);
        WSTAT(WS_RAY, s_ray);
        WSTAT(WS_CYC_START, t_c - t_start);
        WSTAT(WS_CYC_C, t_c1 - t_c);
        WSTAT(WS_CYC_RAY, t_ray - t_c1);
        WSTAT(WS_CYC_EMIT, t_end - t_ray);
        WSTAT(WS_UB0, __float_as_uint(st_ub0));
        WSTAT(WS_UBEND, __float_as_uint(ube));
        WSTAT(WS_LIST, o1 - o0);
        WSTAT(WS_IDEAL_ENTRIES, s_il);
        WSTAT(WS_IDEAL_FACES, s_if);
        WSTAT(WS_DEAD, nf.n_dead);
    }
    if (!BRICK && defer != nullptr) { STAT(4, 1); STAT(5, t_end - t_start); }
#endif
}

template <int PPW, bool BRICK>
__global__ void __launch_bounds__(SW_T, PPW == 32 ? 8 : 0) k_sdf_warp(const float4 *__restrict__ xyz4, const int32_t *__restrict__ perm,
                                                   int64_t N, MeshView m, float *__restrict__ rec,
                                                   int32_t *__restrict__ face, int32_t *__restrict__ defer,
                                                   int32_t *__restrict__ ndefer) {
    static_assert(!BRICK || PPW == 32, "brick lists serve dense lattices: 32 points per warp");
    extern __shared__ __align__(16) unsigned char smem_raw[];
    SdfSmem<PPW, BRICK> &S = reinterpret_cast<SdfSmem<PPW, BRICK> *>(smem_raw)[threadIdx.x >> 5];
    const bool listed = !BRICK && defer != nullptr;
    const int64_t nw = listed ? (int64_t)*ndefer : (N + PPW - 1) / PPW;
    for (int64_t i = (int64_t)blockIdx.x * (SW_T / 32) + (threadIdx.x >> 5); i < nw; i += (int64_t)gridDim.x * (SW_T / 32))
        sdf_warp<PPW, BRICK>(listed ? (int64_t)defer[i] : i, S, xyz4, perm, N, m, rec, face, defer, ndefer);
}

__global__ void k_brick_centres(MeshView m) {
    const int b = blockIdx.x * blockDim.x + threadIdx.x;
    if (b >= NBRICK) return;
    float4 lo, hi;
    brick_box(b, lo, hi);
    m.bxyz[b] = make_float4(0.5f * (lo.x + hi.x), 0.5f * (lo.y + hi.y), 0.5f * (lo.z + hi.z), 0.f);
    m.bperm[b] = b;
}

template <class Take, class Put>
__device__ __forceinline__ int block_gather(int n, int *s_n, Take &&take, Put &&put) {
    __syncthreads();
    for (int i = threadIdx.x; i < n; i += blockDim.x) {
        float key;
        int tag;
        if (take(i, key, tag)) put(atomicAdd(s_n, 1), key, tag);
    }
    __syncthreads();
    return *s_n;
}

__device__ __forceinline__ unsigned long long key_tag(float key, int tag) {
    return (unsigned long long)__float_as_uint(key) << 32 | (unsigned)tag;
}

template <class Put>
__device__ __forceinline__ void rank_sort(const unsigned long long *s_kt, int n, Put &&put) {
    for (int i = threadIdx.x; i < n; i += blockDim.x) {
        const unsigned long long x = s_kt[i];
        int r = 0;
        for (int j = 0; j < n; ++j) r += s_kt[j] < x;
        put(r, i);
    }
}

__device__ __forceinline__ void brick_plane(const MeshView &m, int b, float4 lo, float4 hi, NearestFace<32> &nf) {
    const Tri t = load_tri(m.tri + 3 * (size_t)__ldg(m.bface + b));
    float d[8], sx = 0.f, sy = 0.f, sz = 0.f;
    for (int i = 0; i < 8; ++i) {
        const V3 c = mk3(i & 1 ? hi.x : lo.x, i & 2 ? hi.y : lo.y, i & 4 ? hi.z : lo.z);
        d[i] = sqrtf(tri_sqdist(c, t.a, t.ab, t.ac)) * 1.00001f + 1e-6f;
        sx += i & 1 ? d[i] : -d[i];
        sy += i & 2 ? d[i] : -d[i];
        sz += i & 4 ? d[i] : -d[i];
    }
    const float h = 0.5f * BRICK_W;
    nf.g = mk3(fminf(fmaxf(sx / (8.f * h), -1.f), 1.f), fminf(fmaxf(sy / (8.f * h), -1.f), 1.f),
               fminf(fmaxf(sz / (8.f * h), -1.f), 1.f));
    float beta = -FLT_MAX;
    for (int i = 0; i < 8; ++i)
        beta = fmaxf(beta, d[i] - ((i & 1 ? nf.g.x : -nf.g.x) + (i & 2 ? nf.g.y : -nf.g.y) + (i & 4 ? nf.g.z : -nf.g.z)) * h);
    nf.beta = beta;
}

__device__ __forceinline__ bool brick_face(const MeshView &m, const unsigned short *leaves, int j, float4 lo, float4 hi,
                                           const NearestFace<32> &nf, int &k, float &key) {
    k = 4 * (int)leaves[j / 4] + (j & 3);
    if (k >= m.F) return false;
    const float4 s = __ldg(m.sph_s + k);
    const float4 *tp = m.tri_s + 3 * (size_t)k;
    if (nf.beats(s, __ldg(tp), __ldg(tp + 1), __ldg(tp + 2), lo, hi)) return false;
    const float gap = sqrtf(box_dist2(mk3(s.x, s.y, s.z), lo, hi)) * 0.99999f - s.w - 1e-6f;
    key = gap > 0.f ? gap * gap : 0.f;
    return true;
}

template <bool FILL>
__global__ void __launch_bounds__(128) k_brick_faces(MeshView m, int64_t fcap) {
    static_assert(BRICK_MAX_FACES <= BRICK_MAX_LEAVES, "the face stage reuses the leaf array");
    static_assert(4 * BRICK_MAX_LEAVES <= 65536, "candidate positions are 16-bit tags");
    __shared__ unsigned short s_leaf[BRICK_MAX_LEAVES];
    __shared__ unsigned long long s_kt[FILL ? BRICK_MAX_LEAVES : 1];
    __shared__ int s_n[2];
    if (FILL && (m.hdr->brick_overflow || m.foff[NBRICK] > fcap)) return;
    if (threadIdx.x == 0) s_n[0] = s_n[1] = 0;
    const int b = blockIdx.x;
    float4 lo, hi;
    brick_box(b, lo, hi);
    float ub;
    if (FILL) {
        ub = m.bub[b];
    } else {
        const float4 cc = m.bxyz[b];
        const Tri t = load_tri(m.tri + 3 * (size_t)m.bface[b]);
        const float d = tri_sqdist(mk3(cc.x, cc.y, cc.z), t.a, t.ab, t.ac);
        ub = (sqrtf(d) + BRICK_HALF_DIAG) * 1.00001f + 1e-6f;
    }
    const float ub2 = ub * ub;
    const int n = block_gather(m.lvl_cnt[0], &s_n[0], [&](int l, float &key, int &tag) {
        key = leaf_key(m, l, lo, hi);
        tag = l;
        return key <= ub2;
    }, [&](int at, float key, int tag) {
        if (at >= BRICK_MAX_LEAVES) return;
        if (FILL) s_kt[at] = key_tag(key, tag);
        else s_leaf[at] = (unsigned short)tag;
    });
    NearestFace<32> nf(mk3(0.f, 0.f, 0.f), 1e-6f, 1e-7f);
    brick_plane(m, b, lo, hi, nf);
    if constexpr (!FILL) {
        const bool fits = n <= BRICK_MAX_LEAVES && m.F <= 65535;
        int cnt = 0, k;
        float key;
        if (fits)
            for (int j = threadIdx.x; j < 4 * n; j += blockDim.x) cnt += brick_face(m, s_leaf, j, lo, hi, nf, k, key);
        cnt = __reduce_add_sync(0xffffffffu, cnt);
        if ((threadIdx.x & 31) == 0) atomicAdd(&s_n[1], cnt);
        __syncthreads();
        if (threadIdx.x == 0) {
            m.bub[b] = ub;
            m.foff[b] = s_n[1];
            if (!fits || s_n[1] > BRICK_MAX_FACES) m.hdr->brick_overflow = 1;
            if (b == 0) m.foff[NBRICK] = 0;
        }
    } else {
        rank_sort(s_kt, n, [&](int r, int i) { s_leaf[r] = (unsigned short)s_kt[i]; });
        const int f0 = m.foff[b];
        const int nkept = block_gather(4 * n, &s_n[1], [&](int j, float &key, int &tag) {
            int k;
            tag = j;
            return brick_face(m, s_leaf, j, lo, hi, nf, k, key);
        }, [&](int at, float key, int tag) { if (at < BRICK_MAX_FACES) s_kt[at] = key_tag(key, tag); });
        rank_sort(s_kt, nkept, [&](int r, int i) {
            const unsigned long long x = s_kt[i];
            const int j = (int)(x & 0xffffu);
            m.flist[f0 + r] = (unsigned short)(4 * s_leaf[j / 4] + (j & 3));
            m.fkey[f0 + r] = __uint_as_float((unsigned)(x >> 32));
        });
    }
}

__global__ void k_brick_done(MeshView m, int64_t fcap) {
    if (m.foff[NBRICK] > fcap) m.hdr->brick_overflow = 1;
    m.hdr->brick_built = 1;
}

__global__ void __launch_bounds__(256) k_sdf_brute(const float *__restrict__ pts, int64_t sc, int64_t sn,
                                                   int64_t N, Calib cb, MeshView m,
                                                   float *__restrict__ rec, int32_t *__restrict__ face) {
    __shared__ float4 tile[3 * 256];
    int64_t i = (int64_t)blockIdx.x * blockDim.x + threadIdx.x;
    bool live = i < N;
    V3 p = mk3(0.f, 0.f, 0.f);
    if (live) p = load_point(pts, sc, sn, i, cb);
    float best = FLT_MAX;
    int bi = 0, hits = 0;
    for (int f0 = 0; f0 < m.F; f0 += 256) {
        int nf = min(256, m.F - f0);
        __syncthreads();
        for (int k = threadIdx.x; k < 3 * nf; k += 256) tile[k] = m.tri[3 * (size_t)f0 + k];
        __syncthreads();
        if (live) {
            for (int k = 0; k < nf; ++k) {
                float4 r0 = tile[3 * k], r1 = tile[3 * k + 1], r2 = tile[3 * k + 2];
                V3 a = mk3(r0.x, r0.y, r0.z), ab = mk3(r0.w, r1.x, r1.y), ac = mk3(r1.z, r1.w, r2.x);
                float d = tri_sqdist(p, a, ab, ac);
                if (d < best) { best = d; bi = f0 + k; }
                hits += ray_hit_px(p, a, ab, ac);
            }
        }
    }
    if (live) emit_record(p, bi, best, hits, m, rec, face, i);
}

static int64_t g_sdf_ppw32_from = 6000000, g_sdf_ppw8_from = 300000;
static int g_sdf_ppw_force = 0;
static int g_sdf_bricks = 1;
static int64_t g_brick_max_entries = 0;

static std::mutex g_brick_mu;
static std::unordered_set<const void *> g_brick_ready;
static int64_t g_brick_builds = 0;

void bricks_forget(const MeshView &m) {
    std::lock_guard<std::mutex> lk(g_brick_mu);
    g_brick_ready.erase(m.hdr);
}

struct SdfWs {
    float4 *xyz4;
    int32_t *bid, *perm, *count, *offset;
    int32_t *defer, *ndefer;
    void *scan_ws;
};
static SdfWs carve_sdf(Carver &c, int64_t N) {
    SdfWs w;
    w.xyz4 = c.take<float4>((size_t)N);
    w.bid = c.take<int32_t>((size_t)N);
    w.perm = c.take<int32_t>((size_t)N);
    w.count = c.take<int32_t>(NBIN + 1);
    w.offset = c.take<int32_t>(NBIN + 1);
    w.defer = c.take<int32_t>((size_t)(N + 31) / 32);
    w.ndefer = c.take<int32_t>(1);
    w.scan_ws = c.take<char>(scan_ws_bytes(NBIN + 1));
    return w;
}

static int build_bricks(const MeshView &m, cudaStream_t stream) {
    const int64_t fcap = g_brick_max_entries > 0 ? std::min(g_brick_max_entries, m.face_cap) : m.face_cap;
    k_brick_centres<<<NBRICK / 256, 256, 0, stream>>>(m);
    ICON_LAUNCHED();
    k_sdf_warp<1, false><<<NBRICK / (SW_T / 32), SW_T, sdf_smem_bytes<1, false>(), stream>>>(
        m.bxyz, m.bperm, NBRICK, m, m.brec, m.bface, nullptr, nullptr);
    ICON_LAUNCHED();
    k_brick_faces<false><<<NBRICK, 128, 0, stream>>>(m, fcap);
    ICON_LAUNCHED();
    const int rc = scan_exclusive_i32(m.foff, m.foff, NBRICK + 1, nullptr, m.scan_ws, stream);
    if (rc) return rc;
    k_brick_faces<true><<<NBRICK, 128, 0, stream>>>(m, fcap);
    ICON_LAUNCHED();
    k_brick_done<<<1, 1, 0, stream>>>(m, fcap);
    ICON_LAUNCHED();
    return ICON_OK;
}
size_t sdf_ws_bytes(int64_t N) {
    Carver c(nullptr);
    carve_sdf(c, N);
    return c.total();
}

Calib make_calib(const float *h) {
    Calib cb;
    for (int r = 0; r < 3; ++r) {
        for (int k = 0; k < 3; ++k) cb.r[3 * r + k] = h[4 * r + k];
        cb.t[r] = h[4 * r + 3];
    }
    return cb;
}

int run_sdf(const float *points, int64_t sc, int64_t sn, int64_t N, const float *h_calib,
            const MeshView &m, float *rec, int32_t *face, void *ws, float4 **xyz4_out,
            cudaStream_t stream) {
    Carver c(ws);
    SdfWs w = carve_sdf(c, N);
    Calib cb = make_calib(h_calib);
    profile_mark(0, stream);
    ICON_CUDA(cudaMemsetAsync(w.count, 0, sizeof(int32_t) * (NBIN + 1), stream));
    const unsigned nblk = (unsigned)((N + 255) / 256);
    k_points_bin<<<nblk, 256, 0, stream>>>(points, sc, sn, N, cb, w.xyz4, w.bid, w.count);
    ICON_LAUNCHED();
    int rc = scan_exclusive_i32(w.count, w.offset, NBIN + 1, nullptr, w.scan_ws, stream);
    if (rc) return rc;
    ICON_CUDA(cudaMemsetAsync(w.count, 0, sizeof(int32_t) * (NBIN + 1), stream));
    k_points_scatter<<<nblk, 256, 0, stream>>>(w.bid, N, w.offset, w.count, w.perm);
    ICON_LAUNCHED();
    static bool attr_set[ICON_MAX_DEVICES] = {};
    if (device_needs_setup(attr_set)) {
#define ICON_SDF_ATTR(P, B) ICON_CUDA(cudaFuncSetAttribute(k_sdf_warp<P, B>, cudaFuncAttributeMaxDynamicSharedMemorySize, \
                                                           (int)sdf_smem_bytes<P, B>()))
        ICON_SDF_ATTR(32, true); ICON_SDF_ATTR(32, false); ICON_SDF_ATTR(16, false); ICON_SDF_ATTR(8, false);
        ICON_SDF_ATTR(4, false); ICON_SDF_ATTR(2, false); ICON_SDF_ATTR(1, false);
#undef ICON_SDF_ATTR
    }
    profile_mark(1, stream);
    int ppw = N >= g_sdf_ppw32_from ? 32 : (N >= g_sdf_ppw8_from ? 8 : 1);
    if (g_sdf_ppw_force) ppw = g_sdf_ppw_force;
    const int wpb = SW_T / 32;
    const int64_t nwarps = (N + ppw - 1) / ppw;
    const unsigned nblk_w = (unsigned)((nwarps + wpb - 1) / wpb);
#define ICON_SDF_LAUNCH(P) k_sdf_warp<P, false><<<nblk_w, SW_T, sdf_smem_bytes<P, false>(), stream>>>( \
        w.xyz4, w.perm, N, m, rec, face, nullptr, nullptr)
    if (ppw == 32 && g_sdf_bricks) {
        bool build;
        {
            std::lock_guard<std::mutex> lk(g_brick_mu);
            build = g_brick_ready.insert(m.hdr).second;
        }
        if (build) {
            rc = build_bricks(m, stream);
            std::lock_guard<std::mutex> lk(g_brick_mu);
            if (rc) { g_brick_ready.erase(m.hdr); return rc; }
            ++g_brick_builds;
        }
        ICON_CUDA(cudaMemsetAsync(w.ndefer, 0, sizeof(int32_t), stream));
        k_sdf_warp<32, true><<<nblk_w, SW_T, sdf_smem_bytes<32, true>(), stream>>>(
            w.xyz4, w.perm, N, m, rec, face, w.defer, w.ndefer);
        ICON_LAUNCHED();
        const unsigned nblk_d = (unsigned)std::min<int64_t>(nblk_w, (int64_t)device_sm_count() * 16);
        k_sdf_warp<32, false><<<nblk_d, SW_T, sdf_smem_bytes<32, false>(), stream>>>(
            w.xyz4, w.perm, N, m, rec, face, w.defer, w.ndefer);
    } else {
        switch (ppw) {
            case 32: ICON_SDF_LAUNCH(32); break;
            case 16: ICON_SDF_LAUNCH(16); break;
            case 8: ICON_SDF_LAUNCH(8); break;
            case 4: ICON_SDF_LAUNCH(4); break;
            case 2: ICON_SDF_LAUNCH(2); break;
            default: ICON_SDF_LAUNCH(1); break;
        }
    }
#undef ICON_SDF_LAUNCH
    ICON_LAUNCHED();
    profile_mark(2, stream);
    if (xyz4_out) *xyz4_out = w.xyz4;
    return ICON_OK;
}

__global__ void k_points_only(const float *__restrict__ pts, int64_t sc, int64_t sn, int64_t N, Calib cb,
                              float4 *__restrict__ xyz4) {
    int64_t i = (int64_t)blockIdx.x * blockDim.x + threadIdx.x;
    if (i >= N) return;
    V3 p = load_point(pts, sc, sn, i, cb);
    float in_cube = (p.x > -1.f && p.x < 1.f && p.y > -1.f && p.y < 1.f && p.z > -1.f && p.z < 1.f) ? 1.f : 0.f;
    xyz4[i] = make_float4(p.x, p.y, p.z, in_cube);
}

int run_points_only(const float *points, int64_t sc, int64_t sn, int64_t N, const float *h_calib,
                    float4 *xyz4, cudaStream_t stream) {
    Calib cb = make_calib(h_calib);
    k_points_only<<<(unsigned)((N + 255) / 256), 256, 0, stream>>>(points, sc, sn, N, cb, xyz4);
    ICON_LAUNCHED();
    return ICON_OK;
}

}

using namespace icon;

#ifdef ICON_SDF_STATS
extern "C" int icon_debug_sdf_stats(unsigned long long *out, int reset) {
    cudaMemcpyFromSymbol(out, icon::g_stats, sizeof(unsigned long long) * 8);
    if (reset) { unsigned long long z[8] = {0}; cudaMemcpyToSymbol(icon::g_stats, z, sizeof(z)); }
    return 0;
}

extern "C" int icon_debug_sdf_warp_stats(unsigned *dev_buf) {
    cudaMemcpyToSymbol(icon::g_wstat, &dev_buf, sizeof(dev_buf));
    return 0;
}
#endif

extern "C" int icon_set_sdf_policy(int force_ppw, int64_t ppw8_from, int64_t ppw32_from) {
    ICON_CHECK_ARG(force_ppw >= 0 && force_ppw <= 32 && (force_ppw & (force_ppw - 1)) == 0, "icon_set_sdf_policy: ppw in {0,1,2,4,8,16,32}");
    icon::g_sdf_ppw_force = force_ppw;
    if (ppw8_from >= 0) icon::g_sdf_ppw8_from = ppw8_from;
    if (ppw32_from >= 0) icon::g_sdf_ppw32_from = ppw32_from;
    return ICON_OK;
}

extern "C" int icon_set_sdf_bricks(int enable, int64_t max_entries) {
    ICON_CHECK_ARG(enable == 0 || enable == 1, "icon_set_sdf_bricks: enable must be 0 or 1");
    icon::g_sdf_bricks = enable;
    icon::g_brick_max_entries = max_entries > 0 ? max_entries : 0;
    return ICON_OK;
}

extern "C" int icon_sdf_brick_info(const void *mesh_ws, int V, int F, int64_t *out) {
    ICON_CHECK_ARG(mesh_ws && out && V > 0 && F > 0, "icon_sdf_brick_info: bad argument");
    MeshView m = mesh_view(mesh_ws, V, F);
    MeshHeader h;
    int32_t total = 0;
    ICON_CUDA(cudaDeviceSynchronize());
    ICON_CUDA(cudaMemcpy(&h, m.hdr, sizeof(h), cudaMemcpyDeviceToHost));
    if (h.brick_built) ICON_CUDA(cudaMemcpy(&total, m.foff + NBRICK, sizeof(total), cudaMemcpyDeviceToHost));
    out[0] = h.brick_built;
    out[1] = h.brick_overflow;
    out[2] = total;
    out[3] = m.face_cap;
    {
        std::lock_guard<std::mutex> lk(icon::g_brick_mu);
        out[4] = icon::g_brick_builds;
    }
    return ICON_OK;
}

extern "C" int icon_sdf_brick_lists(const void *mesh_ws, int V, int F, int64_t *dims, int32_t *foff, int32_t *flist,
                                    float *fkey, float *bub, int32_t *bface, float *sph) {
    ICON_CHECK_ARG(mesh_ws && dims && V > 0 && F > 0, "icon_sdf_brick_lists: bad argument");
    MeshView m = mesh_view(mesh_ws, V, F);
    MeshHeader h;
    int32_t total = 0;
    ICON_CUDA(cudaDeviceSynchronize());
    ICON_CUDA(cudaMemcpy(&h, m.hdr, sizeof(h), cudaMemcpyDeviceToHost));
    ICON_CHECK_ARG(h.brick_built, "icon_sdf_brick_lists: the body's brick lists are not built");
    ICON_CHECK_ARG(!h.brick_overflow, "icon_sdf_brick_lists: the body's brick lists overflowed");
    ICON_CUDA(cudaMemcpy(&total, m.foff + NBRICK, sizeof(total), cudaMemcpyDeviceToHost));
    dims[0] = BRICK_AX;
    dims[1] = total;
    if (!foff && !flist && !fkey && !bub && !bface && !sph) return ICON_OK;
    ICON_CHECK_ARG(foff && flist && fkey && bub && bface && sph, "icon_sdf_brick_lists: null array");
    std::vector<int32_t> order((size_t)F);
    std::vector<unsigned short> pos((size_t)total);
    std::vector<float4> sph_s((size_t)F);
    ICON_CUDA(cudaMemcpy(order.data(), m.order, sizeof(int32_t) * F, cudaMemcpyDeviceToHost));
    ICON_CUDA(cudaMemcpy(pos.data(), m.flist, sizeof(unsigned short) * total, cudaMemcpyDeviceToHost));
    ICON_CUDA(cudaMemcpy(sph_s.data(), m.sph_s, sizeof(float4) * F, cudaMemcpyDeviceToHost));
    ICON_CUDA(cudaMemcpy(foff, m.foff, sizeof(int32_t) * (NBRICK + 1), cudaMemcpyDeviceToHost));
    ICON_CUDA(cudaMemcpy(fkey, m.fkey, sizeof(float) * total, cudaMemcpyDeviceToHost));
    ICON_CUDA(cudaMemcpy(bub, m.bub, sizeof(float) * NBRICK, cudaMemcpyDeviceToHost));
    ICON_CUDA(cudaMemcpy(bface, m.bface, sizeof(int32_t) * NBRICK, cudaMemcpyDeviceToHost));
    for (int32_t i = 0; i < total; ++i) flist[i] = order[pos[i]];
    for (int k = 0; k < F; ++k) {
        float *s = sph + 4 * (size_t)order[k];
        s[0] = sph_s[k].x; s[1] = sph_s[k].y; s[2] = sph_s[k].z; s[3] = sph_s[k].w;
    }
    return ICON_OK;
}

extern "C" int icon_sdf_only(const float *points, int64_t stride_c, int64_t stride_n, int64_t N,
                             const float *h_calib, const void *mesh_ws, int V, int F, float *rec,
                             int32_t *face, void *ws, size_t ws_bytes, icon_stream_t stream_) {
    cudaStream_t stream = (cudaStream_t)stream_;
    ICON_CHECK_ARG(N >= 0 && N < (int64_t)INT32_MAX, "icon_sdf_only: N=%lld out of range", (long long)N);
    if (N == 0) return ICON_OK;
    ICON_CHECK_ARG(points && h_calib && mesh_ws && rec && ws, "icon_sdf_only: null pointer");
    if (ws_bytes < sdf_ws_bytes(N)) {
        set_error("icon_sdf_only: workspace %zu < %zu", ws_bytes, sdf_ws_bytes(N));
        return ICON_ENOSPC;
    }
    MeshView m = mesh_view(mesh_ws, V, F);
    return run_sdf(points, stride_c, stride_n, N, h_calib, m, rec, face, ws, nullptr, stream);
}

extern "C" int icon_sdf_bruteforce(const float *points, int64_t stride_c, int64_t stride_n, int64_t N,
                                   const float *h_calib, const void *mesh_ws, int V, int F, float *rec,
                                   int32_t *face, icon_stream_t stream_) {
    cudaStream_t stream = (cudaStream_t)stream_;
    if (N == 0) return ICON_OK;
    ICON_CHECK_ARG(points && h_calib && mesh_ws && rec, "icon_sdf_bruteforce: null pointer");
    MeshView m = mesh_view(mesh_ws, V, F);
    Calib cb = make_calib(h_calib);
    k_sdf_brute<<<(unsigned)((N + 255) / 256), 256, 0, stream>>>(points, stride_c, stride_n, N, cb, m, rec, face);
    ICON_LAUNCHED();
    return ICON_OK;
}
```

include/icon_b200.h:

```cpp
#ifndef ICON_B200_H
#define ICON_B200_H

#include <stddef.h>
#include <stdint.h>

#ifdef __cplusplus
extern "C" {
#endif

#define ICON_OK 0
#define ICON_EINVAL (-1)
#define ICON_ECUDA (-2)
#define ICON_ENOSPC (-3)

#define ICON_PRIOR_ICON 0
#define ICON_PRIOR_PIFU 1
#define ICON_PRIOR_PAMIR 2

typedef void *icon_stream_t;

int icon_version(void);
const char *icon_last_error(void);
int64_t icon_launch_count(void);

int icon_profile_enable(int on);
int icon_profile_last_query(float *h_ms);

size_t icon_smpl_workspace_bytes(int V, int F);
int icon_smpl_prepare(const float *verts, const int64_t *faces, const float *cmap,
                      const float *vis, int V, int F, void *mesh_ws, size_t mesh_ws_bytes,
                      icon_stream_t stream);

#define ICON_MLP_PACKED_FLOATS (16 * 512 + 512 + 512 * 256 + 256 + 272 * 128 + 128 + 144 + 1)
#define ICON_MLP_TC_BYTES (32768 + 8 * 65536 + 4 * 32768 + 8192 + (512 + 256 + 128 + 144 + 4) * 4)
int icon_set_mlp_impl(int impl);
int icon_get_mlp_impl(void);

size_t icon_query_workspace_bytes(int64_t N, int F, int prior);
int icon_query(int prior, const float *points, int64_t stride_c, int64_t stride_n, int64_t N,
               const float *h_calib, const float *feat, int C, int H, int W,
               const float *vol_feat, int VD, const void *mesh_ws, int V, int F,
               const float *mlp_packed, const void *mlp_tc, int c0, float sdf_clip, float *out,
               void *ws, size_t ws_bytes, icon_stream_t stream);

#define ICON_FEAT_CMAP 1
#define ICON_FEAT_NORM 2
#define ICON_FEAT_VIS 4
#define ICON_FEAT_ALL (ICON_FEAT_CMAP | ICON_FEAT_NORM | ICON_FEAT_VIS)
int icon_query_feats(int prior, const float *points, int64_t stride_c, int64_t stride_n, int64_t N,
                     const float *h_calib, const float *feat, int C, int H, int W,
                     const float *vol_feat, int VD, const void *mesh_ws, int V, int F,
                     const float *mlp_packed, const void *mlp_tc, int c0, float sdf_clip, int smpl_feats,
                     float *out, void *ws, size_t ws_bytes, icon_stream_t stream);

int icon_set_sdf_policy(int force_ppw, int64_t ppw8_from, int64_t ppw32_from);
int icon_set_sdf_bricks(int enable, int64_t max_entries);
int icon_sdf_brick_info(const void *mesh_ws, int V, int F, int64_t *out);
int icon_sdf_brick_lists(const void *mesh_ws, int V, int F, int64_t *dims, int32_t *foff, int32_t *flist,
                         float *fkey, float *bub, int32_t *bface, float *sph);

int icon_sdf_only(const float *points, int64_t stride_c, int64_t stride_n, int64_t N,
                  const float *h_calib, const void *mesh_ws, int V, int F, float *rec,
                  int32_t *face, void *ws, size_t ws_bytes, icon_stream_t stream);
int icon_sdf_bruteforce(const float *points, int64_t stride_c, int64_t stride_n, int64_t N,
                        const float *h_calib, const void *mesh_ws, int V, int F, float *rec,
                        int32_t *face, icon_stream_t stream);
int icon_face_tree_read(const void *mesh_ws, int V, int F, int32_t *order, float *tri_s, float *sph_s, float *nodes);
size_t icon_mesh_workspace_bytes(int V, int F);
int icon_mesh_prepare(const float *verts, const int64_t *faces, int V, int F, void *mesh_ws, size_t mesh_ws_bytes,
                      icon_stream_t stream);
int icon_mesh_distance(const float *points, int64_t N, const void *mesh_ws, int V, int F, float *out_sqdist,
                       int32_t *out_face, icon_stream_t stream);
size_t icon_mesh_sample_workspace_bytes(int count);
int icon_mesh_sample(const float *verts, const int64_t *faces, int V, int F, const void *mesh_ws, int count,
                     uint64_t seed, float *out_points, int32_t *out_face, int32_t *out_count, void *ws,
                     size_t ws_bytes, icon_stream_t stream);
size_t icon_prt_workspace_bytes(int V, int D, int K);
int icon_prt(const void *mesh_ws, int Vm, int F, const double *origins, const double *normals, int V, double delta,
             const double *dirs, const double *sh, int D, int K, double w, double *prt_out, uint32_t *hit_bits,
             void *ws, size_t ws_bytes, icon_stream_t stream);

int icon_mlp_only(const float *feature, int c0, int64_t N, const float *mlp_packed,
                  const void *mlp_tc, float *out, icon_stream_t stream);


int icon_display(const float *occ, int R, uint8_t *out , icon_stream_t stream);
int icon_grid_upsample(const float *occ_in, const uint8_t *done_in, int R_in, float balance,
                       float *occ_out, uint8_t *boundary, uint8_t *done_out,
                       icon_stream_t stream);
int icon_grid_dilate(const uint8_t *mask, int R, int k, uint8_t *tmp, uint8_t *out_xyz,
                     icon_stream_t stream);
size_t icon_compact_workspace_bytes(int R);
int icon_grid_compact(const uint8_t *mask_xyz, uint8_t *done, int R, int R_last,
                      const float *h_bmin, const float *h_bmax, float *points, int64_t *indices,
                      int64_t capacity, int64_t *d_count, void *ws, size_t ws_bytes,
                      icon_stream_t stream);
int icon_grid_scatter(float *occ, const int64_t *indices, const float *values, int64_t n,
                      icon_stream_t stream);
int icon_grid_init_points(int R0, int R_last, const float *h_bmin, const float *h_bmax,
                          float *points, icon_stream_t stream);
int icon_grid_count_above(const float *occ, int64_t n, float balance, int64_t *d_count,
                          icon_stream_t stream);

size_t icon_mc_workspace_bytes(int R, int padded);
int icon_mc_count(const float *occ, int R, double iso, int padded, void *ws, size_t ws_bytes,
                  int64_t *d_counts, icon_stream_t stream);
int icon_mc_emit(const float *occ, int R, double iso, int padded, const void *ws, void *verts,
                 int64_t *faces, int64_t n_verts, int64_t n_tris, icon_stream_t stream);

size_t icon_voxelize_workspace_bytes(int res);
int icon_voxelize(const float *verts, int NV, int NVsurf, const float *codes, const int32_t *tets, int NT,
                  int res, float sigma, float *out, void *ws, size_t ws_bytes, icon_stream_t stream);

size_t icon_visibility_workspace_bytes(int image_size);
int icon_visibility(const float *xyz, int V, const int64_t *faces, int F, int image_size, float *vis,
                    void *ws, size_t ws_bytes, icon_stream_t stream);

size_t icon_vertex_normals_workspace_bytes(int V, int F);
int icon_vertex_normals(const double *verts, int V, const int64_t *faces, int F, float *out, void *ws,
                        size_t ws_bytes, icon_stream_t stream);
size_t icon_normal_render_workspace_bytes(int V, int F, int width, int height);
int icon_normal_render(const float *verts, const float *norms, int V, const int64_t *faces, int F,
                       const float *h_model, int width, int height, float *out_rgba, int32_t *out_face,
                       void *ws, size_t ws_bytes, icon_stream_t stream);

#define ICON_DR_PRT 0
#define ICON_DR_COLOR 1
typedef struct {
    int mode, F, V, Vn, Vt, Va;
    const float *pos, *nrm, *uv, *attr;
    const int64_t *f_pos, *f_nrm, *f_uv, *f_attr;
    const uint8_t *tex;
    int tex_w, tex_h;
} icon_dr_mesh;
size_t icon_dataset_render_workspace_bytes(int F, int width, int height, int samples);
int icon_dataset_render(const icon_dr_mesh *mesh, const float *h_view, int width, int height, int samples, float *out,
                        void *ws, size_t ws_bytes, icon_stream_t stream);
size_t icon_dataset_texture_bytes(int w, int h);
int icon_dataset_texture(const uint8_t *rgb, int w, int h, uint8_t *tex, size_t tex_bytes, icon_stream_t stream);

size_t icon_area_vertex_normals_workspace_bytes(int V, int F);
int icon_area_vertex_normals(const float *verts, int V, const int64_t *faces, int F, float *out, void *ws,
                             size_t ws_bytes, icon_stream_t stream);
size_t icon_area_vertex_normals_backward_workspace_bytes(int V, int F);
int icon_area_vertex_normals_backward(const float *verts, int V, const int64_t *faces, int F,
                                      const float *grad_normals, float *grad_verts, void *ws, size_t ws_bytes,
                                      icon_stream_t stream);
size_t icon_mesh_views_workspace_bytes(int V, int F, int S, int A);
int icon_mesh_views(const float *verts, const float *colors, int V, const int64_t *faces, int F,
                    const float *h_view_mats, int A, int S, uint8_t *out, int32_t *face_out, float *rgb_out,
                    void *ws, size_t ws_bytes, icon_stream_t stream);
#define ICON_RENDER_NORMAL 0
#define ICON_RENDER_SILHOUETTE 1
size_t icon_mesh_render_state_bytes(int mode, int S, int A);
size_t icon_mesh_render_workspace_bytes(int mode, int backward, int V, int F, int S, int A);
int icon_mesh_render_forward(int mode, const float *verts, const float *colors, int V, const int64_t *faces, int F,
                             const float *h_view_mats, int A, int S, float *out, void *state, size_t state_bytes,
                             void *ws, size_t ws_bytes, icon_stream_t stream);
int icon_mesh_render_backward(int mode, const float *verts, const float *colors, int V, const int64_t *faces, int F,
                              const float *h_view_mats, int A, int S, const float *grad_out, const void *state,
                              size_t state_bytes, float *grad_verts, float *grad_colors, void *ws, size_t ws_bytes,
                              icon_stream_t stream);

typedef struct {
    int V, F, E;
    const int64_t *faces;
    int64_t *edges;
    int64_t *face_to_edge;
    int32_t *vert_off;
    int32_t *vert_edges;
    int32_t *edge_off;
    int32_t *edge_entries;
    int32_t *corner_off;
    int32_t *vert_corners;
} icon_mesh_topology;
size_t icon_mesh_topology_workspace_bytes(int V, int F);
int icon_mesh_topology_count(const int64_t *faces, int V, int F, int64_t *h_E, void *ws, size_t ws_bytes,
                             icon_stream_t stream);
int icon_mesh_topology_build(const icon_mesh_topology *t, void *ws, size_t ws_bytes, icon_stream_t stream);
size_t icon_vertex_edges_workspace_bytes(int V, int E);
int icon_vertex_edges(const int64_t *edges, int E, int V, int32_t *vert_off, int32_t *vert_edges, void *ws,
                      size_t ws_bytes, icon_stream_t stream);
size_t icon_mesh_priors_workspace_bytes(int V, int F, int E, int backward);
int icon_mesh_priors_forward(const icon_mesh_topology *t, const float *verts, float *out_edge, float *out_nc,
                             float *out_lap, void *ws, size_t ws_bytes, icon_stream_t stream);
int icon_mesh_priors_backward(const icon_mesh_topology *t, const float *verts, const float *g_edge, const float *g_nc,
                              const float *g_lap, float *grad_verts, void *ws, size_t ws_bytes, icon_stream_t stream);
size_t icon_remesh_workspace_bytes(int V, int F, int E);
int icon_remesh_compact(const double *verts, int V, const int64_t *faces, int F, double *out_verts,
                        int64_t *out_faces, int64_t *d_count, void *ws, size_t ws_bytes, icon_stream_t stream);
int icon_remesh_classify(const icon_mesh_topology *t, const double *verts, void *ws, size_t ws_bytes,
                         icon_stream_t stream);
int icon_remesh_smooth_step(const icon_mesh_topology *t, const double *verts, double *out, void *ws,
                            size_t ws_bytes, icon_stream_t stream);
int icon_remesh_midpoints(const icon_mesh_topology *t, const double *verts, float *out, icon_stream_t stream);
int icon_remesh_select(int op, const icon_mesh_topology *t, const double *verts, double L, int adaptive,
                       const float *sqdist, double dlim2, int64_t *d_count, void *ws, size_t ws_bytes,
                       icon_stream_t stream);
int icon_remesh_apply(int op, const icon_mesh_topology *t, const double *verts, int W, double *out_verts,
                      int64_t *out_faces, void *ws, size_t ws_bytes, icon_stream_t stream);
int icon_remesh_relax(const icon_mesh_topology *t, const double *verts, const float *normals, double *out,
                      float *out32, int32_t *moved, void *ws, size_t ws_bytes, icon_stream_t stream);
int icon_remesh_reproject(const double *verts, int V, const int32_t *moved, const int32_t *face,
                          const double *ref_verts, const int64_t *ref_faces, double *out, icon_stream_t stream);
int icon_local_affine_forward(const float *A, const float *b, const float *x, int N, const int64_t *edges, int E,
                              float *out, float *w_diff, float *w_rigid, icon_stream_t stream);
int icon_local_affine_backward(const float *A, const float *b, const float *x, int N, const int64_t *edges, int E,
                               const int32_t *vert_off, const int32_t *vert_edges, const float *g_out,
                               const float *g_diff, const float *g_rigid, float *grad_A, float *grad_b, float *grad_x,
                               icon_stream_t stream);

typedef struct {
    int V, J, NB;
    int parents[64];
    const float *v_template;
    const float *shapedirs;
    const float *posedirs;
    const float *J_regressor;
    const float *lbs_weights;
    double *J_template;
    double *J_dirs;
} icon_lbs_model;
size_t icon_lbs_prepare_workspace_bytes(int V, int J, int NB);
int icon_lbs_prepare(icon_lbs_model *m, const int64_t *h_parents, int posedirs_rows, void *ws, size_t ws_bytes,
                     icon_stream_t stream);
size_t icon_lbs_state_bytes(int B, int V, int J, int NB);
size_t icon_lbs_workspace_bytes(int B, int V, int J, int NB, int backward);
int icon_lbs_forward(const icon_lbs_model *m, int B, const float *betas, const float *pose, int pose2rot, float *verts,
                     float *joints, void *state, size_t state_bytes, void *ws, size_t ws_bytes, icon_stream_t stream);
int icon_lbs_backward(const icon_lbs_model *m, int B, const void *state, size_t state_bytes, const float *grad_verts,
                      const float *grad_joints, float *grad_betas, float *grad_pose, void *ws, size_t ws_bytes,
                      icon_stream_t stream);

#define ICON_HEADS_LUT_ROWS 79
#define ICON_HEADS_MAX_CHAIN 8
typedef struct {
    int V, J, R;
    int Ls, Ld, E, nchain;
    int chain[ICON_HEADS_MAX_CHAIN];
    const float *regressor;
    int *vid;
    float *bc;
    int *joint_reg;
    int *reg_joint;
    int *inc_off;
    int *inc;
} icon_smplx_heads;
int icon_smplx_heads_prepare(icon_smplx_heads *h, const int64_t *h_faces, int F, const int64_t *h_lmk_faces_idx,
                             const float *h_lmk_bary, int Ls, const int64_t *h_dyn_faces_idx, const float *h_dyn_bary,
                             int Ld, const int64_t *h_face_ids, const float *h_bcs, int E, const int64_t *h_source,
                             const int64_t *h_target, int S, const int64_t *h_chain, int nchain,
                             icon_stream_t stream);
size_t icon_smplx_heads_state_bytes(int B, int V, int R);
int icon_smplx_heads_forward(const icon_smplx_heads *h, int B, const float *verts, const float *joints_lbs,
                             const float *pose, float *landmarks, float *joints, int *rows, void *state,
                             size_t state_bytes, icon_stream_t stream);
int icon_smplx_heads_backward(const icon_smplx_heads *h, int B, const int *rows, const float *grad_landmarks,
                              const float *grad_joints, float *grad_verts, float *grad_joints_lbs,
                              icon_stream_t stream);

#define ICON_TETRA_JOINTS 24
#define ICON_TETRA_BETAS 10
#define ICON_TETRA_PAD_V 8000
#define ICON_TETRA_PAD_F 25100
typedef struct {
    int V, N, T, nnz;
    int parents[ICON_TETRA_JOINTS];
    const double *v_template;
    const double *shapedirs;
    const double *posedirs;
    const double *weights;
    const int *jr_off;
    const int *jr_col;
    const double *jr_val;
} icon_tetra_model;
int icon_tetra_prepare(icon_tetra_model *m, const int64_t *h_parents, int J, int posedirs_cols, int nbetas);
size_t icon_tetra_state_bytes(void);
int icon_tetra_forward(const icon_tetra_model *m, const float *rotmats, float *aa, const float *betas,
                       const float *trans, const float *scale, float *voxel_verts, void *state, size_t state_bytes,
                       icon_stream_t stream);

int icon_normalize_mask(const float *x, const float *image, float *y, int N, int Cimg, int64_t HW,
                        icon_stream_t stream);
int icon_conv3d(const float *x, const float *w, const float *scale, const float *shift, const float *res, float *y,
                int Cin, int Cout, int D, int H, int W, int k, int stride, int pad, int dil, int relu,
                icon_stream_t stream);
size_t icon_conv_nhwc_workspace_bytes(int N, int Ht, int Wt, int Cout, int splits);
int icon_conv_nhwc(const void *a_hi, const void *a_lo, const int64_t *dims, const int64_t *strides, const void *wt_packed,
                   int wt_chunks, const float *wt_scale, const float *bias, float *out, int OHf, int OWf, int Cs, int co_off,
                   int Cout, int N,
                   int Ht, int Wt, int osy, int osx, int ooy, int oox, int nplanes, int ntaps, const int *taps, int cpt,
                   int n_tile, int splits, double *stats, void *ws, size_t ws_bytes, icon_stream_t stream);
int icon_norm_finalize(const double *stats, const float *gamma, const float *beta, float *scale_shift, int N, int C,
                       int groups, double count, float eps, icon_stream_t stream);
int icon_act_nhwc(const float *x, int Cs_in, int ci_off, const float *scale_shift, const double *stats, const float *gamma,
                  const float *beta, int groups, float eps, const float *res, void *hi, void *lo, float *f32, int N, int H,
                  int W, int C, int Cp, int halo, int s2d, int relu, icon_stream_t stream);
int icon_splitk_instnorm_act(const float *partial, int splits, const float *bias, const float *res, void *hi, void *lo,
                             float *f32, int N, int H, int W, int C, int Cp, int halo, int relu, float eps,
                             icon_stream_t stream);
int icon_col2im7(const float *P, const float *bias, float *y, int N, int H, int W, int Cout, int Ps, int act,
                 icon_stream_t stream);
int icon_ew_nhwc(int mode, const float *a, const float *b, const float *c, float *y, double *stats, int N, int H, int W,
                 int C, icon_stream_t stream);
int icon_nchw_to_nhwc(const float *x, float *y, double *stats, int N, int C, int64_t HW, icon_stream_t stream);
int icon_nhwc_to_nchw(const float *x, float *y, int N, int C, int Cs, int c_off, int64_t HW, icon_stream_t stream);
int icon_stem_pack(const float *x, void *hi, void *lo, int N, int Cin, int H, int W, int Cp8, int Wp, int Hrows, int sy,
                   int reflect, icon_stream_t stream);
size_t icon_clean_mesh_workspace_bytes(int64_t nv, int64_t nf);
int icon_clean_mesh_count(const int64_t *faces, int64_t nv, int64_t nf, void *ws, size_t ws_bytes, int64_t *d_counts,
                          icon_stream_t stream);
int icon_clean_mesh_emit(const void *verts, int verts_f64, const int64_t *faces, int64_t nv, int64_t nf, const void *ws,
                         float *out_verts, int32_t *out_faces, icon_stream_t stream);

size_t icon_garment_labels_workspace_bytes(int S);
int icon_garment_labels(const double *recon_verts, int V, const double *smpl_verts, int S, const uint8_t *h_smpl_parts,
                        uint8_t *labels, void *ws, size_t ws_bytes, icon_stream_t stream);
size_t icon_garment_face_mask_workspace_bytes(int V, int npoly);
int icon_garment_face_mask(const double *verts, int V, const int64_t *faces, int F, const uint8_t *labels,
                           uint32_t remove_parts, const double *poly_xy, int NP, const int32_t *h_poly_off, int npoly,
                           uint8_t *face_mask, int32_t *kept_count, void *ws, size_t ws_bytes, icon_stream_t stream);

#ifdef __cplusplus
}
#endif
#endif
```

Baseline: 643.3.

## Recompute query points in-kernel, sort points in scatter, tile-based outlier ranking

Drops the materialised xyz4 buffer for the MLP and recomputes the calibrated point from raw input inside the MLP kernels. Removes the separate points-only pass and the bid array: the scatter kernel recomputes the bin itself and writes the sorted xyz4 plus index directly, so the SDF kernel reads points contiguously. The outlier handling now gets a compact per-point class byte from the SDF emit, replacing the full-N flag scan with a per-tile popcount count, a small scan and a ballot-based rank kernel. The aim is fewer launches and less global traffic, at the cost of redundant strided point loads in the MLP. A debug readback entry point is also added.

```diff
diff --git a/icon_b200/_C.py b/icon_b200/_C.py
--- a/icon_b200/_C.py
+++ b/icon_b200/_C.py
@@ -28,6 +28,7 @@
                         _vp, _vp, _sz, _vp]),
     "icon_query_feats": (_i, [_i, _vp, _i64, _i64, _i64, _vp, _vp, _i, _i, _i, _vp, _i, _vp, _i, _i, _vp, _vp, _i, _f,
                               _i, _vp, _vp, _sz, _vp]),
+    "icon_query_outlier_rank": (_i, [_vp, _i64, _vp, _vp, _vp]),
     "icon_set_sdf_policy": (_i, [_i, _i64, _i64]),
     "icon_set_sdf_bricks": (_i, [_i, _i64]),
     "icon_sdf_brick_info": (_i, [_vp, _i, _i, _vp]),
diff --git a/icon_b200/csrc/mlp.cu b/icon_b200/csrc/mlp.cu
--- a/icon_b200/csrc/mlp.cu
+++ b/icon_b200/csrc/mlp.cu
@@ -46,7 +46,7 @@
         if (MODE == 3) {
             for (int r = grp; r < 16; r += 4) x0s[r * MP + pl] = (live && r < c0) ? q.raw[(size_t)r * q.N + pi] : 0.f;
         } else {
-            float4 xyz = live ? q.xyz4[pi] : make_float4(0.f, 0.f, 0.f, 0.f);
+            float4 xyz = live ? query_point(q.pts, q.sc, q.sn, pi, q.cb) : make_float4(0.f, 0.f, 0.f, 0.f);
             if (MODE == 0) {
                 const bool has_vis = q.feats & ICON_FEAT_VIS;
                 const int d = has_vis ? q.C / 2 : q.C;
@@ -245,24 +245,85 @@
             for (int w = 0; w < 8; ++w) s += red[w * MP + tid];
             for (int j = 0; j < 16; ++j) s = fmaf(__ldg(W + OFF_W3 + 128 + j), x0s[j * MP + tid], s);
             s += __ldg(W + OFF_B3);
-            float in_cube = (MODE == 3) ? 1.f : q.xyz4[pi].w;
+            float in_cube = (MODE == 3) ? 1.f : query_point(q.pts, q.sc, q.sn, pi, q.cb).w;
             q.out[pi] = in_cube * s;
         }
     }
 }
 
-__global__ void k_outlier_flag(const float *__restrict__ rec, int64_t N, float clip, int32_t *__restrict__ flag) {
-    int64_t i = (int64_t)blockIdx.x * blockDim.x + threadIdx.x;
-    if (i < N) flag[i] = fabsf(rec[8 * i]) >= clip ? 1 : 0;
-}
-__global__ void k_outlier_signs(const float *__restrict__ rec, int64_t N, float clip,
-                                const int32_t *__restrict__ krank, int8_t *__restrict__ signs) {
-    int64_t i = (int64_t)blockIdx.x * blockDim.x + threadIdx.x;
-    if (i < N) {
-        float s = rec[8 * i];
-        if (fabsf(s) >= clip) signs[krank[i]] = s > 0.f ? 1 : -1;
-    }
-}
+constexpr int RANK_T = 256, RANK_TILE = 32 * RANK_T;
+
+__device__ __forceinline__ int rank_load(const uint8_t *__restrict__ cls, int64_t N, int64_t t0, int tid, uint4 (&v)[2]) {
+    const int64_t b = t0 + 32 * tid;
+    if (b + 32 <= N) {
+        v[0] = *(const uint4 *)(cls + b);
+        v[1] = *(const uint4 *)(cls + b + 16);
+    } else {
+        uint32_t w[8] = {};
+        for (int j = 0; j < 32; ++j)
+            if (b + j < N) w[j / 4] |= (uint32_t)cls[b + j] << (8 * (j % 4));
+        v[0] = make_uint4(w[0], w[1], w[2], w[3]);
+        v[1] = make_uint4(w[4], w[5], w[6], w[7]);
+    }
+    constexpr uint32_t BIT0 = 0x01010101u * CLS_OUTLIER;
+    return __popc(v[0].x & BIT0) + __popc(v[0].y & BIT0) + __popc(v[0].z & BIT0) + __popc(v[0].w & BIT0) +
+           __popc(v[1].x & BIT0) + __popc(v[1].y & BIT0) + __popc(v[1].z & BIT0) + __popc(v[1].w & BIT0);
+}
+
+__global__ void __launch_bounds__(RANK_T) k_outlier_count(const uint8_t *__restrict__ cls, int64_t N,
+                                                          int32_t *__restrict__ tile_cnt) {
+    __shared__ int s_warp[RANK_T / 32];
+    uint4 v[2];
+    const int cnt = __reduce_add_sync(0xffffffffu, rank_load(cls, N, (int64_t)blockIdx.x * RANK_TILE, threadIdx.x, v));
+    if ((threadIdx.x & 31) == 0) s_warp[threadIdx.x >> 5] = cnt;
+    __syncthreads();
+    if (threadIdx.x == 0) {
+        int total = 0;
+#pragma unroll
+        for (int k = 0; k < RANK_T / 32; ++k) total += s_warp[k];
+        tile_cnt[blockIdx.x] = total;
+    }
+}
+
+__global__ void __launch_bounds__(RANK_T) k_outlier_rank(const uint8_t *__restrict__ cls, int64_t N,
+                                                         const int32_t *__restrict__ tile_off,
+                                                         int32_t *__restrict__ krank, int8_t *__restrict__ signs) {
+    __shared__ __align__(16) uint8_t s_cls[RANK_TILE];
+    __shared__ int8_t s_sign[RANK_TILE];
+    __shared__ int s_warp[RANK_T / 32];
+    const int tid = threadIdx.x, lane = tid & 31, wid = tid >> 5;
+    const int64_t t0 = (int64_t)blockIdx.x * RANK_TILE;
+    uint4 v[2];
+    const int cnt = __reduce_add_sync(0xffffffffu, rank_load(cls, N, t0, tid, v));
+    reinterpret_cast<uint4 *>(s_cls)[2 * tid] = v[0];
+    reinterpret_cast<uint4 *>(s_cls)[2 * tid + 1] = v[1];
+    if (lane == 0) s_warp[wid] = cnt;
+    __syncthreads();
+    int before = 0, total = 0;
+#pragma unroll
+    for (int k = 0; k < RANK_T / 32; ++k) {
+        before += k < wid ? s_warp[k] : 0;
+        total += s_warp[k];
+    }
+    const int excl = tile_off[blockIdx.x];
+    int run = before;
+    const unsigned lt = (1u << lane) - 1u;
+#pragma unroll 4
+    for (int i = 0; i < 32; ++i) {
+        const int at = wid * 1024 + 32 * i + lane;
+        const unsigned c = s_cls[at];
+        const bool out = c & CLS_OUTLIER;
+        const unsigned m = __ballot_sync(0xffffffffu, out);
+        const int r = run + __popc(m & lt);
+        if (t0 + at < N) krank[t0 + at] = excl + r;
+        if (out) s_sign[r] = c & CLS_POSITIVE ? 1 : -1;
+        run += __popc(m);
+    }
+    __syncthreads();
+    for (int k = tid; k < total; k += RANK_T) signs[excl + k] = s_sign[k];
+}
+
+static int outlier_rank_tiles(int64_t N) { return (int)((N + RANK_TILE - 1) / RANK_TILE); }
 
 constexpr size_t MLP_SMEM = (16 * MP + 10240 + 256 * MP) * sizeof(float);
 
@@ -299,18 +360,17 @@
 
 size_t sdf_ws_bytes(int64_t N);
 int run_sdf(const float *points, int64_t sc, int64_t sn, int64_t N, const float *h_calib, const MeshView &m,
-            float *rec, int32_t *face, void *ws, float4 **xyz4_out, cudaStream_t stream);
-int run_points_only(const float *points, int64_t sc, int64_t sn, int64_t N, const float *h_calib,
-                    float4 *xyz4, cudaStream_t stream);
+            float *rec, int32_t *face, uint8_t *cls, float clip, void *ws, cudaStream_t stream);
 
 struct QueryWs {
     void *sdf_ws;
     float *rec;
+    uint8_t *cls;
     int32_t *krank;
     int8_t *signs;
     int64_t *d_K;
+    int32_t *tiles;
     void *scan_ws;
-    float4 *xyz4;
 };
 
 static QueryWs carve_query(Carver &c, int64_t N, int prior) {
@@ -318,12 +378,12 @@
     if (prior == ICON_PRIOR_ICON) {
         w.sdf_ws = c.take<char>(sdf_ws_bytes(N));
         w.rec = c.take<float>((size_t)N * 8);
+        w.cls = c.take<uint8_t>((size_t)N);
         w.krank = c.take<int32_t>((size_t)N);
         w.signs = c.take<int8_t>((size_t)N);
         w.d_K = c.take<int64_t>(1);
-        w.scan_ws = c.take<char>(scan_ws_bytes(N));
-    } else {
-        w.xyz4 = c.take<float4>((size_t)N);
+        w.tiles = c.take<int32_t>((size_t)outlier_rank_tiles(N));
+        w.scan_ws = c.take<char>(scan_ws_bytes(outlier_rank_tiles(N)));
     }
     return w;
 }
@@ -373,6 +433,7 @@
     QueryParams q{};
     q.feat = feat; q.C = C; q.H = H; q.W = W; q.vol = vol_feat; q.VD = VD;
     q.mlp = mlp_packed; q.c0 = c0; q.clip = sdf_clip; q.out = out; q.N = N;
+    q.pts = points; q.sc = stride_c; q.sn = stride_n; q.cb = make_calib(h_calib);
     if (prior == ICON_PRIOR_ICON) {
         ICON_CHECK_ARG(mesh_ws && V > 0 && F > 0, "icon_query: icon prior needs a prepared body mesh");
         ICON_CHECK_ARG((smpl_feats & ~ICON_FEAT_ALL) == 0, "icon_query: smpl_feats mask %d has bits outside ICON_FEAT_ALL",
@@ -385,30 +446,28 @@
                        vs ? "C/2" : "C", tail, C, c0);
         q.feats = smpl_feats;
         MeshView m = mesh_view(mesh_ws, V, F);
-        float4 *xyz4 = nullptr;
-        int rc = run_sdf(points, stride_c, stride_n, N, h_calib, m, w.rec, nullptr, w.sdf_ws, &xyz4, stream);
+        int rc = run_sdf(points, stride_c, stride_n, N, h_calib, m, w.rec, nullptr, cm ? w.cls : nullptr, sdf_clip,
+                         w.sdf_ws, stream);
         if (rc) return rc;
         if (cm) {
-            unsigned nb = (unsigned)((N + 255) / 256);
-            k_outlier_flag<<<nb, 256, 0, stream>>>(w.rec, N, sdf_clip, w.krank);
+            const int nt = outlier_rank_tiles(N);
+            k_outlier_count<<<nt, RANK_T, 0, stream>>>(w.cls, N, w.tiles);
             ICON_LAUNCHED();
-            rc = scan_exclusive_i32(w.krank, w.krank, N, w.d_K, w.scan_ws, stream);
+            rc = scan_exclusive_i32(w.tiles, w.tiles, nt, w.d_K, w.scan_ws, stream);
             if (rc) return rc;
-            k_outlier_signs<<<nb, 256, 0, stream>>>(w.rec, N, sdf_clip, w.krank, w.signs);
+            k_outlier_rank<<<nt, RANK_T, 0, stream>>>(w.cls, N, w.tiles, w.krank, w.signs);
             ICON_LAUNCHED();
             q.krank = w.krank; q.signs = w.signs; q.d_K = w.d_K;
         }
-        q.xyz4 = xyz4; q.rec = w.rec;
+        q.rec = w.rec;
         profile_mark(3, stream);
         rc = launch_any<0>(q, mlp_tc, stream);
         profile_mark(4, stream);
         return rc;
     }
     profile_mark(0, stream);
-    int rc = run_points_only(points, stride_c, stride_n, N, h_calib, w.xyz4, stream);
-    if (rc) return rc;
     profile_mark(1, stream); profile_mark(2, stream); profile_mark(3, stream);
-    q.xyz4 = w.xyz4;
+    int rc;
     if (prior == ICON_PRIOR_PIFU) {
         ICON_CHECK_ARG(C + 1 == c0, "icon_query: pifu prior expects c0 = C + 1 (C=%d c0=%d)", C, c0);
         rc = launch_any<1>(q, mlp_tc, stream);
@@ -423,6 +482,18 @@
     }
     set_error("icon_query: unknown prior %d", prior);
     return ICON_EINVAL;
+}
+
+extern "C" int icon_query_outlier_rank(const void *ws, int64_t N, int32_t *krank, int8_t *signs, int64_t *K) {
+    ICON_CHECK_ARG(ws && krank && signs && K && N > 0 && N < (int64_t)INT32_MAX, "icon_query_outlier_rank: bad argument");
+    Carver c(const_cast<void *>(ws));
+    const QueryWs w = carve_query(c, N, ICON_PRIOR_ICON);
+    ICON_CUDA(cudaDeviceSynchronize());
+    ICON_CUDA(cudaMemcpy(K, w.d_K, sizeof(int64_t), cudaMemcpyDeviceToHost));
+    ICON_CHECK_ARG(*K >= 0 && *K <= N, "icon_query_outlier_rank: no outlier rank in this workspace (K=%lld)", (long long)*K);
+    ICON_CUDA(cudaMemcpy(krank, w.krank, sizeof(int32_t) * (size_t)N, cudaMemcpyDeviceToHost));
+    ICON_CUDA(cudaMemcpy(signs, w.signs, (size_t)*K, cudaMemcpyDeviceToHost));
+    return ICON_OK;
 }
 
 extern "C" int icon_set_mlp_impl(int impl) {
diff --git a/icon_b200/csrc/mlp_tc.cu b/icon_b200/csrc/mlp_tc.cu
--- a/icon_b200/csrc/mlp_tc.cu
+++ b/icon_b200/csrc/mlp_tc.cu
@@ -61,7 +61,7 @@
 __device__ __forceinline__ void gather_point(const QueryParams &q, int64_t pi, float *xf) {
 #pragma unroll
     for (int j = 0; j < 15; ++j) xf[j * TC_M] = 0.f;
-    float in_cube = 1.f;
+    xf[15 * TC_M] = 1.f;
     if (pi < q.N) {
         if (MODE == 3) {
             const int c0 = q.c0;
@@ -69,8 +69,8 @@
             for (int j = 0; j < 15; ++j)
                 if (j < c0) xf[j * TC_M] = q.raw[(size_t)j * q.N + pi];
         } else {
-            const float4 xyz = q.xyz4[pi];
-            in_cube = xyz.w;
+            const float4 xyz = query_point(q.pts, q.sc, q.sn, pi, q.cb);
+            xf[15 * TC_M] = xyz.w;
             if (MODE == 0) {
                 const bool has_vis = q.feats & ICON_FEAT_VIS;
                 const int d = has_vis ? q.C / 2 : q.C;
@@ -132,7 +132,6 @@
             }
         }
     }
-    xf[15 * TC_M] = in_cube;
 }
 
 template <int MODE>
diff --git a/icon_b200/csrc/query_common.cuh b/icon_b200/csrc/query_common.cuh
--- a/icon_b200/csrc/query_common.cuh
+++ b/icon_b200/csrc/query_common.cuh
@@ -3,8 +3,28 @@
 
 namespace icon {
 
+struct Calib {
+    float r[9];
+    float t[3];
+};
+Calib make_calib(const float *h);
+
+__device__ __forceinline__ float4 query_point(const float *__restrict__ pts, int64_t sc, int64_t sn, int64_t i,
+                                              const Calib &cb) {
+    const float px = pts[i * sn], py = pts[sc + i * sn], pz = pts[2 * sc + i * sn];
+    const float x = fmaf(cb.r[2], pz, fmaf(cb.r[1], py, cb.r[0] * px)) + cb.t[0];
+    const float y = fmaf(cb.r[5], pz, fmaf(cb.r[4], py, cb.r[3] * px)) + cb.t[1];
+    const float z = fmaf(cb.r[8], pz, fmaf(cb.r[7], py, cb.r[6] * px)) + cb.t[2];
+    const bool in_cube = x > -1.f && x < 1.f && y > -1.f && y < 1.f && z > -1.f && z < 1.f;
+    return make_float4(x, y, z, in_cube ? 1.f : 0.f);
+}
+
+constexpr uint8_t CLS_OUTLIER = 1, CLS_POSITIVE = 2;
+
 struct QueryParams {
-    const float4 *xyz4;
+    const float *pts;
+    int64_t sc, sn;
+    Calib cb;
     const float *rec;
     const int32_t *krank;
     const int8_t *signs;
diff --git a/icon_b200/csrc/sdf.cu b/icon_b200/csrc/sdf.cu
--- a/icon_b200/csrc/sdf.cu
+++ b/icon_b200/csrc/sdf.cu
@@ -9,27 +9,19 @@
 #include "common.cuh"
 #include "face_tree.cuh"
 #include "geom.cuh"
+#include "query_common.cuh"
 
 namespace icon {
 
-struct Calib {
-    float r[9];
-    float t[3];
-};
-
-__device__ __forceinline__ V3 load_point(const float *__restrict__ pts, int64_t sc, int64_t sn,
-                                         int64_t i, const Calib &cb) {
-    float px = pts[i * sn], py = pts[sc + i * sn], pz = pts[2 * sc + i * sn];
-    V3 o;
-    o.x = fmaf(cb.r[2], pz, fmaf(cb.r[1], py, cb.r[0] * px)) + cb.t[0];
-    o.y = fmaf(cb.r[5], pz, fmaf(cb.r[4], py, cb.r[3] * px)) + cb.t[1];
-    o.z = fmaf(cb.r[8], pz, fmaf(cb.r[7], py, cb.r[6] * px)) + cb.t[2];
-    return o;
+__device__ __forceinline__ V3 load_point(const float *__restrict__ pts, int64_t sc, int64_t sn, int64_t i,
+                                         const Calib &cb) {
+    const float4 q = query_point(pts, sc, sn, i, cb);
+    return mk3(q.x, q.y, q.z);
 }
 
 __device__ __forceinline__ void emit_record(V3 p, int bi, float best, int hits, const MeshView &m,
                                             float *__restrict__ rec, int32_t *__restrict__ face,
-                                            int64_t idx) {
+                                            uint8_t *__restrict__ cls, float clip, int64_t idx) {
     Tri t = load_tri(m.tri + 3 * (size_t)bi);
     V3 n = cross3(t.ab, t.ac);
     float s = n.x * n.x + n.y * n.y + n.z * n.z;
@@ -58,6 +50,7 @@
     r[0] = make_float4(sdf, cx, cy, cz);
     r[1] = make_float4(nx, ny, nz, vis);
     if (face) face[idx] = bi;
+    if (cls) cls[idx] = (fabsf(sdf) >= clip ? CLS_OUTLIER : 0) | (sdf > 0.f ? CLS_POSITIVE : 0);
 }
 
 constexpr int SW_T = 128;
@@ -83,17 +76,10 @@
 }
 
 __global__ void k_points_bin(const float *__restrict__ pts, int64_t sc, int64_t sn, int64_t N, Calib cb,
-                             float4 *__restrict__ xyz4, int32_t *__restrict__ bid, int32_t *__restrict__ count) {
+                             int32_t *__restrict__ count) {
     const int64_t i = (int64_t)blockIdx.x * blockDim.x + threadIdx.x;
     const bool live = i < N;
-    int b = -1;
-    if (live) {
-        const V3 p = load_point(pts, sc, sn, i, cb);
-        const float in_cube = (p.x > -1.f && p.x < 1.f && p.y > -1.f && p.y < 1.f && p.z > -1.f && p.z < 1.f) ? 1.f : 0.f;
-        xyz4[i] = make_float4(p.x, p.y, p.z, in_cube);
-        b = bin_of(p);
-        bid[i] = b;
-    }
+    const int b = live ? bin_of(load_point(pts, sc, sn, i, cb)) : -1;
     const unsigned act = __ballot_sync(0xffffffffu, live);
     if (live) {
         const unsigned peers = __match_any_sync(act, b);
@@ -101,19 +87,21 @@
     }
 }
 
-__global__ void k_points_scatter(const int32_t *__restrict__ bid, int64_t N, const int32_t *__restrict__ offset,
-                                 int32_t *__restrict__ cursor, int32_t *__restrict__ perm) {
+__global__ void k_points_scatter(const float *__restrict__ pts, int64_t sc, int64_t sn, int64_t N, Calib cb,
+                                 int32_t *__restrict__ cursor, float4 *__restrict__ xyz4, int32_t *__restrict__ idx) {
     const int64_t i = (int64_t)blockIdx.x * blockDim.x + threadIdx.x;
     const bool live = i < N;
-    const int b = live ? bid[i] : -1;
+    const float4 q = live ? query_point(pts, sc, sn, i, cb) : make_float4(0.f, 0.f, 0.f, 0.f);
+    const int b = live ? bin_of(mk3(q.x, q.y, q.z)) : -1;
     const unsigned act = __ballot_sync(0xffffffffu, live);
     if (live) {
         const unsigned peers = __match_any_sync(act, b);
         const int lane = threadIdx.x & 31, leader = __ffs(peers) - 1;
         int base = 0;
         if (lane == leader) base = atomicAdd(&cursor[b], __popc(peers));
-        base = __shfl_sync(peers, base, leader);
-        perm[offset[b] + base + __popc(peers & ((1u << lane) - 1u))] = (int32_t)i;
+        const int at = __shfl_sync(peers, base, leader) + __popc(peers & ((1u << lane) - 1u));
+        xyz4[at] = q;
+        idx[at] = (int32_t)i;
     }
 }
 
@@ -154,9 +142,9 @@
 
 template <int PPW, bool BRICK>
 __device__ __forceinline__ void sdf_warp(int64_t wid, SdfSmem<PPW, BRICK> &S, const float4 *__restrict__ xyz4,
-                                         const int32_t *__restrict__ perm, int64_t N, const MeshView &m,
-                                         float *__restrict__ rec, int32_t *__restrict__ face,
-                                         int32_t *__restrict__ defer, int32_t *__restrict__ ndefer) {
+                                         const int32_t *__restrict__ sidx, int64_t N, const MeshView &m,
+                                         float *__restrict__ rec, int32_t *__restrict__ face, uint8_t *__restrict__ cls,
+                                         float clip, int32_t *__restrict__ defer, int32_t *__restrict__ ndefer) {
     constexpr int REP = 32 / PPW;
     const int lane = threadIdx.x & 31;
     const int sub = lane % PPW, rep_id = lane / PPW;
@@ -164,8 +152,8 @@
     const int64_t pos = pos0 + sub;
     if (pos0 >= N) return;
     const bool live = pos < N;
-    const int64_t idx = perm[live ? pos : pos0];
-    const float4 q = xyz4[idx];
+    const int64_t idx = sidx[live ? pos : pos0];
+    const float4 q = xyz4[live ? pos : pos0];
     const V3 p = mk3(q.x, q.y, q.z);
     const V3 c = mk3(0.5f * (warp_min(p.x) + warp_max(p.x)), 0.5f * (warp_min(p.y) + warp_max(p.y)),
                      0.5f * (warp_min(p.z) + warp_max(p.z)));
@@ -263,7 +251,7 @@
     WCLK(t_ray0);
     t_ray = t_ray0;
 #endif
-    if (live && rep_id == 0) emit_record(p, nf.bi, nf.best, hits, m, rec, face, idx);
+    if (live && rep_id == 0) emit_record(p, nf.bi, nf.best, hits, m, rec, face, cls, clip, idx);
 #ifdef ICON_SDF_STATS
     WCLK(t_end);
     if (BRICK && st_brick >= 0) {
@@ -302,17 +290,17 @@
 }
 
 template <int PPW, bool BRICK>
-__global__ void __launch_bounds__(SW_T, PPW == 32 ? 8 : 0) k_sdf_warp(const float4 *__restrict__ xyz4, const int32_t *__restrict__ perm,
+__global__ void __launch_bounds__(SW_T, PPW == 32 ? 8 : 0) k_sdf_warp(const float4 *__restrict__ xyz4, const int32_t *__restrict__ sidx,
                                                    int64_t N, MeshView m, float *__restrict__ rec,
-                                                   int32_t *__restrict__ face, int32_t *__restrict__ defer,
-                                                   int32_t *__restrict__ ndefer) {
+                                                   int32_t *__restrict__ face, uint8_t *__restrict__ cls, float clip,
+                                                   int32_t *__restrict__ defer, int32_t *__restrict__ ndefer) {
     static_assert(!BRICK || PPW == 32, "brick lists serve dense lattices: 32 points per warp");
     extern __shared__ __align__(16) unsigned char smem_raw[];
     SdfSmem<PPW, BRICK> &S = reinterpret_cast<SdfSmem<PPW, BRICK> *>(smem_raw)[threadIdx.x >> 5];
     const bool listed = !BRICK && defer != nullptr;
     const int64_t nw = listed ? (int64_t)*ndefer : (N + PPW - 1) / PPW;
     for (int64_t i = (int64_t)blockIdx.x * (SW_T / 32) + (threadIdx.x >> 5); i < nw; i += (int64_t)gridDim.x * (SW_T / 32))
-        sdf_warp<PPW, BRICK>(listed ? (int64_t)defer[i] : i, S, xyz4, perm, N, m, rec, face, defer, ndefer);
+        sdf_warp<PPW, BRICK>(listed ? (int64_t)defer[i] : i, S, xyz4, sidx, N, m, rec, face, cls, clip, defer, ndefer);
 }
 
 __global__ void k_brick_centres(MeshView m) {
@@ -476,7 +464,7 @@
             }
         }
     }
-    if (live) emit_record(p, bi, best, hits, m, rec, face, i);
+    if (live) emit_record(p, bi, best, hits, m, rec, face, nullptr, 0.f, i);
 }
 
 static int64_t g_sdf_ppw32_from = 6000000, g_sdf_ppw8_from = 300000;
@@ -495,17 +483,16 @@
 
 struct SdfWs {
     float4 *xyz4;
-    int32_t *bid, *perm, *count, *offset;
+    int32_t *sidx;
+    int32_t *count;
     int32_t *defer, *ndefer;
     void *scan_ws;
 };
 static SdfWs carve_sdf(Carver &c, int64_t N) {
     SdfWs w;
     w.xyz4 = c.take<float4>((size_t)N);
-    w.bid = c.take<int32_t>((size_t)N);
-    w.perm = c.take<int32_t>((size_t)N);
+    w.sidx = c.take<int32_t>((size_t)N);
     w.count = c.take<int32_t>(NBIN + 1);
-    w.offset = c.take<int32_t>(NBIN + 1);
     w.defer = c.take<int32_t>((size_t)(N + 31) / 32);
     w.ndefer = c.take<int32_t>(1);
     w.scan_ws = c.take<char>(scan_ws_bytes(NBIN + 1));
@@ -517,7 +504,7 @@
     k_brick_centres<<<NBRICK / 256, 256, 0, stream>>>(m);
     ICON_LAUNCHED();
     k_sdf_warp<1, false><<<NBRICK / (SW_T / 32), SW_T, sdf_smem_bytes<1, false>(), stream>>>(
-        m.bxyz, m.bperm, NBRICK, m, m.brec, m.bface, nullptr, nullptr);
+        m.bxyz, m.bperm, NBRICK, m, m.brec, m.bface, nullptr, 0.f, nullptr, nullptr);
     ICON_LAUNCHED();
     k_brick_faces<false><<<NBRICK, 128, 0, stream>>>(m, fcap);
     ICON_LAUNCHED();
@@ -545,7 +532,7 @@
 }
 
 int run_sdf(const float *points, int64_t sc, int64_t sn, int64_t N, const float *h_calib,
-            const MeshView &m, float *rec, int32_t *face, void *ws, float4 **xyz4_out,
+            const MeshView &m, float *rec, int32_t *face, uint8_t *cls, float clip, void *ws,
             cudaStream_t stream) {
     Carver c(ws);
     SdfWs w = carve_sdf(c, N);
@@ -553,12 +540,11 @@
     profile_mark(0, stream);
     ICON_CUDA(cudaMemsetAsync(w.count, 0, sizeof(int32_t) * (NBIN + 1), stream));
     const unsigned nblk = (unsigned)((N + 255) / 256);
-    k_points_bin<<<nblk, 256, 0, stream>>>(points, sc, sn, N, cb, w.xyz4, w.bid, w.count);
-    ICON_LAUNCHED();
-    int rc = scan_exclusive_i32(w.count, w.offset, NBIN + 1, nullptr, w.scan_ws, stream);
+    k_points_bin<<<nblk, 256, 0, stream>>>(points, sc, sn, N, cb, w.count);
+    ICON_LAUNCHED();
+    int rc = scan_exclusive_i32(w.count, w.count, NBIN + 1, nullptr, w.scan_ws, stream);
     if (rc) return rc;
-    ICON_CUDA(cudaMemsetAsync(w.count, 0, sizeof(int32_t) * (NBIN + 1), stream));
-    k_points_scatter<<<nblk, 256, 0, stream>>>(w.bid, N, w.offset, w.count, w.perm);
+    k_points_scatter<<<nblk, 256, 0, stream>>>(points, sc, sn, N, cb, w.count, w.xyz4, w.sidx);
     ICON_LAUNCHED();
     static bool attr_set[ICON_MAX_DEVICES] = {};
     if (device_needs_setup(attr_set)) {
@@ -575,7 +561,7 @@
     const int64_t nwarps = (N + ppw - 1) / ppw;
     const unsigned nblk_w = (unsigned)((nwarps + wpb - 1) / wpb);
 #define ICON_SDF_LAUNCH(P) k_sdf_warp<P, false><<<nblk_w, SW_T, sdf_smem_bytes<P, false>(), stream>>>( \
-        w.xyz4, w.perm, N, m, rec, face, nullptr, nullptr)
+        w.xyz4, w.sidx, N, m, rec, face, cls, clip, nullptr, nullptr)
     if (ppw == 32 && g_sdf_bricks) {
         bool build;
         {
@@ -590,11 +576,11 @@
         }
         ICON_CUDA(cudaMemsetAsync(w.ndefer, 0, sizeof(int32_t), stream));
         k_sdf_warp<32, true><<<nblk_w, SW_T, sdf_smem_bytes<32, true>(), stream>>>(
-            w.xyz4, w.perm, N, m, rec, face, w.defer, w.ndefer);
+            w.xyz4, w.sidx, N, m, rec, face, cls, clip, w.defer, w.ndefer);
         ICON_LAUNCHED();
         const unsigned nblk_d = (unsigned)std::min<int64_t>(nblk_w, (int64_t)device_sm_count() * 16);
         k_sdf_warp<32, false><<<nblk_d, SW_T, sdf_smem_bytes<32, false>(), stream>>>(
-            w.xyz4, w.perm, N, m, rec, face, w.defer, w.ndefer);
+            w.xyz4, w.sidx, N, m, rec, face, cls, clip, w.defer, w.ndefer);
     } else {
         switch (ppw) {
             case 32: ICON_SDF_LAUNCH(32); break;
@@ -608,24 +594,6 @@
 #undef ICON_SDF_LAUNCH
     ICON_LAUNCHED();
     profile_mark(2, stream);
-    if (xyz4_out) *xyz4_out = w.xyz4;
-    return ICON_OK;
-}
-
-__global__ void k_points_only(const float *__restrict__ pts, int64_t sc, int64_t sn, int64_t N, Calib cb,
-                              float4 *__restrict__ xyz4) {
-    int64_t i = (int64_t)blockIdx.x * blockDim.x + threadIdx.x;
-    if (i >= N) return;
-    V3 p = load_point(pts, sc, sn, i, cb);
-    float in_cube = (p.x > -1.f && p.x < 1.f && p.y > -1.f && p.y < 1.f && p.z > -1.f && p.z < 1.f) ? 1.f : 0.f;
-    xyz4[i] = make_float4(p.x, p.y, p.z, in_cube);
-}
-
-int run_points_only(const float *points, int64_t sc, int64_t sn, int64_t N, const float *h_calib,
-                    float4 *xyz4, cudaStream_t stream) {
-    Calib cb = make_calib(h_calib);
-    k_points_only<<<(unsigned)((N + 255) / 256), 256, 0, stream>>>(points, sc, sn, N, cb, xyz4);
-    ICON_LAUNCHED();
     return ICON_OK;
 }
 
@@ -725,7 +693,7 @@
         return ICON_ENOSPC;
     }
     MeshView m = mesh_view(mesh_ws, V, F);
-    return run_sdf(points, stride_c, stride_n, N, h_calib, m, rec, face, ws, nullptr, stream);
+    return run_sdf(points, stride_c, stride_n, N, h_calib, m, rec, face, nullptr, 0.f, ws, stream);
 }
 
 extern "C" int icon_sdf_bruteforce(const float *points, int64_t stride_c, int64_t stride_n, int64_t N,
diff --git a/include/icon_b200.h b/include/icon_b200.h
--- a/include/icon_b200.h
+++ b/include/icon_b200.h
@@ -52,6 +52,7 @@
                      const float *vol_feat, int VD, const void *mesh_ws, int V, int F,
                      const float *mlp_packed, const void *mlp_tc, int c0, float sdf_clip, int smpl_feats,
                      float *out, void *ws, size_t ws_bytes, icon_stream_t stream);
+int icon_query_outlier_rank(const void *ws, int64_t N, int32_t *krank, int8_t *signs, int64_t *K);
 
 int icon_set_sdf_policy(int force_ppw, int64_t ppw8_from, int64_t ppw32_from);
 int icon_set_sdf_bricks(int enable, int64_t max_entries);
```

Measured after the change: 652.5 (median of 6 runs). 1.4% higher.
